# tigert1998/ray-tracing-cuda

Measured on AMD Instinct MI355X. Metric: Mrays/s, higher is better.
Workload: dtype f32

## Files before the change

### ray-tracing-cuda_amd/csrc/capi.hip

```cpp
#include <hip/hip_runtime.h>
#include <dlfcn.h>
#include <rccl/rccl.h>
#include <string.h>

#include <algorithm>
#include <cmath>
#include <cstdlib>
#include <mutex>
#include <string>
#include <unordered_map>

#include "../../include/rtmi.h"
#include "kernels.h"
#include "scene.h"
#include "xorwow.h"

using namespace rtmi;

static thread_local std::string g_err;
static int fail(int code, const std::string &msg) {
  g_err = msg;
  return code;
}
static int hip_fail(hipError_t e, const char *what) {
// ... 332 lines not shown
  if (!s || !pos || !look_at || !up) return fail(RTMI_ERR_INVALID, "null argument");
  camera_pinhole(*S(s), v3(pos), v3(look_at), v3(up), fov, aspect);
  S(s)->committed = false;
  return RTMI_OK;
}
int rtmi_camera_defocus(rtmi_scene *s, const float pos[3], const float look_at[3], const float up[3], double fov,
                        double aspect, double aperture, double focus_distance) {
  if (!s || !pos || !look_at || !up) return fail(RTMI_ERR_INVALID, "null argument");
  camera_defocus(*S(s), v3(pos), v3(look_at), v3(up), fov, aspect, aperture, focus_distance);
  S(s)->committed = false;
  return RTMI_OK;
}
int rtmi_camera_raw(rtmi_scene *s, const float pos[3], const float llc[3], const float horiz[3], const float vert[3]) {
  if (!s || !pos || !llc || !horiz || !vert) return fail(RTMI_ERR_INVALID, "null argument");
  camera_raw(*S(s), v3(pos), v3(llc), v3(horiz), v3(vert));
  S(s)->committed = false;
  return RTMI_OK;
}
int rtmi_camera_set(rtmi_scene *s, const float f[21], int is_defocus, double lens_radius) {
  if (!s || !f) return fail(RTMI_ERR_INVALID, "null argument");
  CameraDev &c = S(s)->cam;
  c.position = v3(f), c.llc = v3(f + 3), c.horizontal = v3(f + 6), c.vertical = v3(f + 9);
  c.u = v3(f + 12), c.v = v3(f + 15);
  S(s)->cam_w = v3(f + 18);
  c.defocus = is_defocus ? 1 : 0;
  c.lens_radius = (float)lens_radius;
  S(s)->has_camera = true;
  S(s)->committed = false;
  return RTMI_OK;
}
int rtmi_camera_update(rtmi_scene *s, const float f[21], int is_defocus, double lens_radius) {
  if (!s || !f) return fail(RTMI_ERR_INVALID, "null argument");
  if (!all_finite(f, 21)) return fail(RTMI_ERR_INVALID, "non-finite camera float");
  Scene *sc = S(s);
  const bool committed = sc->committed;
  if (int rc = rtmi_camera_set(s, f, is_defocus, lens_radius)) return rc;
  if (committed) {
    sc->dev.cam = sc->cam;
    sc->features = sc->cam.defocus ? sc->features | F_DEFOCUS : sc->features & ~(uint32_t)F_DEFOCUS;
    sc->committed = true;
  }
  return RTMI_OK;
}
int rtmi_camera_get(const rtmi_scene *s, float out[21]) {
  if (!s || !out || !S(s)->has_camera) return fail(RTMI_ERR_INVALID, "scene has no camera");
  const CameraDev &c = S(s)->cam;
  const V3 vs[7] = {c.position, c.llc, c.horizontal, c.vertical, c.u, c.v, S(s)->cam_w};
  for (int i = 0; i < 7; i++) out[i * 3] = vs[i].x, out[i * 3 + 1] = vs[i].y, out[i * 3 + 2] = vs[i].z;
  return RTMI_OK;
}

int rtmi_scene_commit(rtmi_scene *sp) {
  if (!sp) return fail(RTMI_ERR_INVALID, "null scene");
  Scene *s = S(sp);
  if (s->list_counts.size() != 1) return fail(RTMI_ERR_INVALID, "a nested list is still open (rtmi_list_end missing)");
  static_assert(RTMI_MAX_MATERIALS == kMaxMats, "rtmi.h and scene_dev.h disagree on the material limit");
  if (s->mats.size() > (size_t)RTMI_MAX_MATERIALS)
    return fail(RTMI_ERR_CAPACITY, "more than RTMI_MAX_MATERIALS (2^24) materials: a triangle's material field has 24 bits");
  if (rtmi_device_count() <= 0) return fail(RTMI_ERR_NO_DEVICE, "no HIP device: librtmi has no CPU fallback");
  free_device(s);
  std::string err = s->flatten();
  if (!err.empty()) return fail(RTMI_ERR_INVALID, err);
  HIP_TRY(hipGetDevice(&s->device));
  s->tex_recs.clear();
  for (const HostTex &t : s->texs) {
    if (!t.image) continue;
    void *d = nullptr;
    size_t pitch = 0;
    HIP_TRY(hipMallocPitch(&d, &pitch, (size_t)t.w * 4, (size_t)t.h));
    s->dev_allocs.push_back(d);
    HIP_TRY(hipMemcpy2D(d, pitch, t.rgba.data(), (size_t)t.w * 4, (size_t)t.w * 4, (size_t)t.h,
                        hipMemcpyHostToDevice));
    TexRec r{};
    r.rgba = reinterpret_cast<const uint8_t *>(d);
    r.height = t.h, r.width = t.w, r.pitch = (int64_t)pitch;
    s->tex_recs.push_back(r);
  }
  SceneDev d{};
  int rc;
  if ((rc = upload(s, s->runs, &d.runs))) return rc;
  if ((rc = upload(s, s->spheres, &d.spheres))) return rc;
  if ((rc = upload(s, s->tris, &d.tris))) return rc;
  if ((rc = upload(s, s->pair_boxes, &d.pair_boxes))) return rc;
  if ((rc = upload(s, s->pair_pts, &d.pair_pts))) return rc;
  if ((rc = upload(s, s->tri_nrm, &d.tri_nrm))) return rc;
  if ((rc = upload(s, s->sph_groups, &d.sph_groups))) return rc;
  if ((rc = upload(s, s->sph_members, &d.sph_members))) return rc;
  d.sph_mag = s->sph_mag;
  d.n_sph_groups = (int)s->sph_groups.size();
  if ((rc = upload(s, s->bvh_recs, &d.bvhs))) return rc;
  if ((rc = upload(s, s->nodes, &d.nodes))) return rc;
  if ((rc = upload(s, s->qnodes, &d.qnodes))) return rc;
  if ((rc = upload(s, s->leaf_paths, &d.leaf_paths))) return rc;
  if ((rc = upload(s, s->tops, &d.tops))) return rc;
  if ((rc = upload(s, s->faces, &d.faces))) return rc;
  if ((rc = upload(s, s->face_uv, &d.face_uv))) return rc;
#ifdef RTMI_CHECK_MARGINS
  if ((rc = upload(s, s->face_of_orig, &d.face_of_orig))) return rc;
#endif
  if ((rc = upload(s, s->mat_recs, &d.mats))) return rc;
  if ((rc = upload(s, s->tex_recs, &d.texs))) return rc;
  d.n_runs = (int)s->runs.size() - 4;
  d.n_pairs = (int)s->pair_pts.size();
  d.list_mag = s->list_mag;
  d.n_mats = (int)s->mat_recs.size();
  d.n_nodes = (int)s->nodes.size();
  d.n_leaf_paths = (int)s->leaf_paths.size();
  d.sub_reserve = s->sub_depth > 0 ? 3 * s->sub_depth + 3 + kMeshFaceSlack : 0;
  d.det_safe = 1;
  for (const HotTri &t : s->tris) {
    const double a = std::sqrt((double)t.e1[0] * t.e1[0] + (double)t.e1[1] * t.e1[1] + (double)t.e1[2] * t.e1[2]);
    const double b = std::sqrt((double)t.e2[0] * t.e2[0] + (double)t.e2[1] * t.e2[1] + (double)t.e2[2] * t.e2[2]);
    if (!(a * b <= 0x1p120)) d.det_safe = 0;
  }
  d.unsigned_colours = 1;
  for (const MatRec &m : s->mat_recs) {
    const float c[3] = {m.r, m.g, m.b};
    for (float x : c) {
      uint32_t bits;
      memcpy(&bits, &x, sizeof(bits));
      if (bits >> 31) d.unsigned_colours = 0;
    }
  }
  d.cam = s->cam;
  s->dev = d;
  QueryDev q{};
  if ((rc = upload(s, s->q_sphere_entry, &q.sphere_entry))) return rc;
  if ((rc = upload(s, s->q_pair_entry, &q.pair_entry))) return rc;
  if ((rc = upload(s, s->q_bvh_entry, &q.bvh_entry))) return rc;
  if ((rc = upload(s, s->q_face_input, &q.face_input))) return rc;
  q.sky_entry = s->q_sky_entry;
  s->qdev = q;
  void *c = nullptr;
  HIP_TRY(hipMalloc(&c, RTMI_COUNTER_WORDS * sizeof(unsigned long long) + 2 * render_params_bytes()));
  s->dev_allocs.push_back(c);
  HIP_TRY(hipMemset(c, 0, RTMI_COUNTER_WORDS * sizeof(unsigned long long)));
  s->d_counters = reinterpret_cast<unsigned long long *>(c);
  HIP_TRY(hipDeviceSynchronize());
  s->committed = true;
  return RTMI_OK;
}

static int flattened(const rtmi_scene *sp, Scene *tmp) {
  *tmp = *S(sp);
  tmp->dev_allocs.clear();
  const std::string err = tmp->flatten();
  return err.empty() ? RTMI_OK : fail(RTMI_ERR_INVALID, err);
}
int rtmi_scene_stats(const rtmi_scene *sp, int64_t out[8]) {
  if (!sp || !out) return fail(RTMI_ERR_INVALID, "null argument");
  Scene tmp;
  if (int rc = flattened(sp, &tmp)) return rc;
  out[0] = (int64_t)tmp.list_counts[0];
  out[1] = (int64_t)tmp.n_spheres;
  out[2] = (int64_t)tmp.n_pgrams;
  out[3] = (int64_t)tmp.n_triangles;
  out[4] = (int64_t)tmp.faces.size();
  out[5] = (int64_t)tmp.nodes.size();
  out[6] = (int64_t)tmp.mat_recs.size();
  out[7] = (int64_t)tmp.texs.size();
  return RTMI_OK;
}

int64_t rtmi_scene_sliver_faces(const rtmi_scene *sp) {
  if (!sp) return fail(RTMI_ERR_INVALID, "null scene");
  Scene tmp;
  if (int rc = flattened(sp, &tmp)) return rc;
  return tmp.sliver_faces;
}

int64_t rtmi_scene_bytes_per_ray(const rtmi_scene *sp) {
  if (!sp) return fail(RTMI_ERR_INVALID, "null scene");
  Scene tmp;
  if (int rc = flattened(sp, &tmp)) return rc;
  return tmp.bytes_per_ray;
}

int64_t rtmi_frame_work_items(const rtmi_frame *f) {
  FrameDev d;
  if (!make_frame(f, &d)) return fail(RTMI_ERR_INVALID, frame_why("bad frame"));
  return d.items;
}
int64_t rtmi_frame_pixel_of(const rtmi_frame *f, int64_t q) {
  FrameDev d;
  if (!make_frame(f, &d) || q < 0 || q >= d.items) return -1;
  return frame_pixel_of(d, d.rank, q);
}
int rtmi_frame_pixel_map(const rtmi_frame *f, int64_t *out) {
  FrameDev d;
  if (!make_frame(f, &d) || !out) return fail(RTMI_ERR_INVALID, frame_why("bad frame"));
  for (int64_t q = 0; q < d.items; q++) out[q] = frame_pixel_of(d, d.rank, q);
  return RTMI_OK;
}
size_t rtmi_states_bytes(const rtmi_frame *f) {
  FrameDev d;
  if (!make_frame(f, &d)) return 0;
  return (size_t)d.items * RTMI_STATE_WORDS * sizeof(uint32_t);
}
size_t rtmi_tiles_bytes(const rtmi_frame *f) {
  FrameDev d;
  if (!make_frame(f, &d)) return 0;
  return (size_t)d.items * 3 * sizeof(float);
}

int rtmi_rng_init(uint64_t seed, const rtmi_frame *f, void *d_states, void *stream) {
  FrameDev d;
  if (!make_frame(f, &d) || !d_states) return fail(RTMI_ERR_INVALID, frame_why("bad rng_init arguments"));
  if (rtmi_device_count() <= 0) return fail(RTMI_ERR_NO_DEVICE, "no HIP device: librtmi has no CPU fallback");
  uint32_t *jump = nullptr;
  int rc = device_jump(&jump);
  if (rc) return rc;
  HIP_TRY(launch_rng_init(seed, d, jump, reinterpret_cast<uint32_t *>(d_states), (hipStream_t)stream));
  return RTMI_OK;
}
int rtmi_rng_init_n(uint64_t seed, uint64_t first, int64_t n, void *d_states, void *stream) {
  if (n < 0 || n > (int64_t)INT32_MAX || (n > 0 && !d_states) || first > (1ull << kJumpBits) ||
      (uint64_t)n > (1ull << kJumpBits) - first)
    return fail(RTMI_ERR_INVALID, "bad rng_init_n arguments (n < 0, n above 2^31 - 1, first + n above 2^40, or null states)");
  if (n == 0) return RTMI_OK;
  if (rtmi_device_count() <= 0) return fail(RTMI_ERR_NO_DEVICE, "no HIP device: librtmi has no CPU fallback");
  uint32_t *jump = nullptr;
  int rc = device_jump(&jump);
  if (rc) return rc;
  FrameDev d{};
  d.items = n;
  HIP_TRY(launch_rng_init(seed, d, jump, reinterpret_cast<uint32_t *>(d_states), (hipStream_t)stream, (int64_t)first));
  return RTMI_OK;
}
int rtmi_rng_host_state(uint64_t seed, uint64_t subsequence, uint32_t state[RTMI_STATE_WORDS]) {
  if (!state) return fail(RTMI_ERR_INVALID, "null state");
  Rng r = host_rng_init(seed, subsequence);
  state[0] = r.d, state[1] = r.v0, state[2] = r.v1, state[3] = r.v2, state[4] = r.v3, state[5] = r.v4;
  return RTMI_OK;
}
float rtmi_rng_host_random_float(float mn, float mx, uint32_t state[RTMI_STATE_WORDS]) {
  Rng r{state[0], state[1], state[2], state[3], state[4], state[5]};
  float x = rng_range(mn, mx, r);
  state[0] = r.d, state[1] = r.v0, state[2] = r.v1, state[3] = r.v2, state[4] = r.v3, state[5] = r.v4;
  return x;
}
int rtmi_rng_set_state(const rtmi_frame *f, void *d_states, int64_t q, const uint32_t state[RTMI_STATE_WORDS],
                       void *stream) {
  FrameDev d;
  if (!make_frame(f, &d) || !d_states || !state || q < 0 || q >= d.items)
    return fail(RTMI_ERR_INVALID, "bad rng_set_state arguments");
  uint32_t *base = reinterpret_cast<uint32_t *>(d_states);
  for (int w = 0; w < RTMI_STATE_WORDS; w++)
    HIP_TRY(hipMemcpyAsync(base + (size_t)w * d.items + q, &state[w], sizeof(uint32_t), hipMemcpyHostToDevice,
                           (hipStream_t)stream));
  HIP_TRY(hipStreamSynchronize((hipStream_t)stream));
  return RTMI_OK;
}
int rtmi_rng_get_state(const rtmi_frame *f, const void *d_states, int64_t q, uint32_t state[RTMI_STATE_WORDS],
                       void *stream) {
  FrameDev d;
  if (!make_frame(f, &d) || !d_states || !state || q < 0 || q >= d.items)
    return fail(RTMI_ERR_INVALID, "bad rng_get_state arguments");
  const uint32_t *base = reinterpret_cast<const uint32_t *>(d_states);
// ... 795 lines not shown
```

### ray-tracing-cuda_amd/csrc/closest_hit.h

```cpp
#pragma once

#ifdef RTMI_CHECK_MARGINS
__device__ inline bool aabb_hit_reference(const BvhNode &nd, V3 o, V3 d, double t_from, double t_to) {
  const float oo[3] = {o.x, o.y, o.z}, dd[3] = {d.x, d.y, d.z};
  for (int i = 0; i < 3; i++) {
    if (dd[i] == 0.f) continue;
    for (int s = 0; s < 2; s++) {
      const float tf = ((s == 0 ? nd.mn[i] : nd.mx[i]) - oo[i]) / dd[i];
      const double t = (double)tf;
      if (t != t || fabs(t) == (double)INFINITY) continue;
      if (!(t_from <= t && t <= t_to)) continue;
      const float pt[3] = {oo[0] + (float)t * dd[0], oo[1] + (float)t * dd[1], oo[2] + (float)t * dd[2]};
      bool inside = true;
      for (int a = 0; a < 3; a++)
        if (a != i && !(nd.mn[a] <= pt[a] && pt[a] <= nd.mx[a])) inside = false;
      if (inside) return true;
    }
  }
  return false;
}
template <typename T>
__device__ inline bool bvh_reference_walk(const SceneDev &sc, const BvhRec &br, V3 o, V3 d, T &t_to, int &face, float &fu,
                                          float &fv) {
  int stk_node[kRefDepthMax + 2], stk_first[kRefDepthMax + 2], stk_n[kRefDepthMax + 2];
  int sp = 1;
  stk_node[0] = br.root, stk_first[0] = 0, stk_n[0] = br.n_faces;
  bool hit = false;
  while (sp > 0) {
    sp--;
    const int node = stk_node[sp], first = stk_first[sp], n = stk_n[sp];
    const BvhNode nd = sc.nodes[node];
    if (node != br.root && !aabb_hit_reference(nd, o, d, 1e-3, (double)t_to)) continue;
    if (nd.right < 0) {
      for (int i = 0; i < n; i++) {
        const int fi = sc.face_of_orig[br.face_base + first + i];
        const FaceRec &f = sc.faces[fi];
        float t = 0.f, u = 0.f, v = 0.f;
        if (tri_test<T>(mk(f.p0[0], f.p0[1], f.p0[2]), mk(f.e1[0], f.e1[1], f.e1[2]), mk(f.e2[0], f.e2[1], f.e2[2]), o, d,
                        t_to, t, u, v))
          t_to = (T)t, face = fi, fu = u, fv = v, hit = true;
      }
    } else if (sp + 2 <= kRefDepthMax + 2) {
      const int mid = (n - 1) / 2;
      stk_node[sp] = nd.right, stk_first[sp] = first + mid + 1, stk_n[sp] = n - mid - 1;
      stk_node[sp + 1] = nd.left, stk_first[sp + 1] = first, stk_n[sp + 1] = mid + 1;
      sp += 2;
    }
  }
  return hit;
}
#endif

template <uint32_t F, bool OCC = false, uint32_t M = 0>
__device__ __forceinline__ Hit closest_hit(const SceneDev &sc, const BvhNode *s_nodes, int lds_nodes, const int *s_paths,
                                           int lds_paths, const float4 *s_pairs, int *ll, uint16_t *cands, int *wl,
                                           unsigned long long *overflow, V3 o, V3 d, bool live, bool count_work
#ifdef RTMI_STATS
                                           , MeshStats &st
#endif
                                           , double t_start = INFINITY, double t_stop = INFINITY, bool *uncertain = nullptr
) {
  constexpr bool DT = (F & F_SPHERE) != 0;
  typedef typename TSel<DT>::type T;
  bool ok = false;
  T t_to = OCC ? (T)t_start : (T)INFINITY;
#define RTMI_DECIDED (OCC && ok && t_to <= (T)t_stop)
  uint32_t win = ID_NONE;
  int32_t aux = 0;
  int32_t work = 0;
  float bu = 0.f, bv = 0.f;

  double sa = 0.0, sa2 = 0.0;
  float saf = 0.f;
  if (F & F_SPHERE) {
    float la = len3(d);
    saf = la * la;
    sa = (double)saf;
    sa2 = 2 * sa;
  }

  const int lane = (int)(threadIdx.x & 63u);
  const bool det_safe = (M & PIN_DET_SAFE) || sc.det_safe != 0;
  const bool cull_list = (F & F_TRIS) && ((M & PIN_LDS_TABLES) || (ll != nullptr && sc.n_pairs >= kCullMinPairs));
  V3 cull_inv = splat(0.f), cull_klo = splat(0.f), cull_khi = splat(0.f);
  if ((F & F_TRIS) && cull_list) {
    const float ix = __builtin_amdgcn_rcpf(d.x), iy = __builtin_amdgcn_rcpf(d.y), iz = __builtin_amdgcn_rcpf(d.z);
    cull_inv = mk(fabsf(d.x) < 1e-30f ? copysignf(1e30f, d.x) : ix, fabsf(d.y) < 1e-30f ? copysignf(1e30f, d.y) : iy,
                  fabsf(d.z) < 1e-30f ? copysignf(1e30f, d.z) : iz);
    const float delta = MESH_DIST_SLACK * (fmaxf(fmaxf(fabsf(o.x), fabsf(o.y)), fabsf(o.z)) + sc.list_mag);
    cull_klo = mk(-(o.x + delta) * cull_inv.x, -(o.y + delta) * cull_inv.y, -(o.z + delta) * cull_inv.z);
    cull_khi = mk(-(o.x - delta) * cull_inv.x, -(o.y - delta) * cull_inv.y, -(o.z - delta) * cull_inv.z);
  }

  for (int ri = 0; ri < sc.n_runs; ri++) {
    if (OCC) {
      live = live && !RTMI_DECIDED;
      if (__builtin_amdgcn_ballot_w64(live) == 0ull) break;
    }
    const i32x4 rv = load_run(sc.runs, ri);
    Run run;
    run.kind = rv[0], run.first = rv[1], run.count = rv[2], run.pad = rv[3];
    if (live && run.kind == RUN_SKY) {
      const T ts = (T)1e9f;
      bool hit = ts <= t_to;
      bool acc = hit && (!ok || ts < t_to);
      ok = ok || acc;
      t_to = acc ? ts : t_to;
      win = acc ? make_id(RUN_SKY, 0) : win;
    }
    if ((F & F_TRIS) && run.kind == RUN_TRIS && cull_list) {
      const int pair0 = run.first >> 1;
      const float lo0 = T_FROM_F * kTimeLo;
      for (int c0 = 0; c0 < run.count; c0 += 32) {
        if (OCC && __builtin_amdgcn_ballot_w64(live && !RTMI_DECIDED) == 0ull) break;
        const int nc = run.count - c0 < 32 ? run.count - c0 : 32;
        const float hi0 = (float)t_to * kTimeHi + kTimeAbs;
        uint32_t mask = 0u;
        RTMI_STAT2(const unsigned long long tc0 = stat_now();)
#define RTMI_CULL_PAIR(bx)                                                                                                      \
  {                                                                                                                             \
    const float t0x = __builtin_fmaf(bx[0], cull_inv.x, cull_klo.x), t1x = __builtin_fmaf(bx[3], cull_inv.x, cull_khi.x); \
    const float t0y = __builtin_fmaf(bx[1], cull_inv.y, cull_klo.y), t1y = __builtin_fmaf(bx[4], cull_inv.y, cull_khi.y); \
    const float t0z = __builtin_fmaf(bx[2], cull_inv.z, cull_klo.z), t1z = __builtin_fmaf(bx[5], cull_inv.z, cull_khi.z); \
    const float en = fmaxf(fmaxf(fminf(t0x, t1x), fminf(t0y, t1y)), fminf(t0z, t1z));                                            \
    const float le = fminf(fminf(fmaxf(t0x, t1x), fmaxf(t0y, t1y)), fmaxf(t0z, t1z));                                            \
    cull_step(mask, fmaxf(lo0, en), fminf(hi0, le));                                                                            \
  }
        f32x8 A = load_pair_box(sc.pair_boxes, pair0 + c0), B;
        int i = 0;
        for (; i + 1 < nc; i += 2) {
          __builtin_amdgcn_s_waitcnt(0xc07f);
          __builtin_amdgcn_sched_barrier(0);
          B = load_pair_box(sc.pair_boxes, pair0 + c0 + i + 1);
          __builtin_amdgcn_sched_barrier(0);
          RTMI_CULL_PAIR(A)
          __builtin_amdgcn_s_waitcnt(0xc07f);
          __builtin_amdgcn_sched_barrier(0);
          A = load_pair_box(sc.pair_boxes, pair0 + c0 + i + 2);
          __builtin_amdgcn_sched_barrier(0);
          RTMI_CULL_PAIR(B)
        }
        if (i < nc) {
          __builtin_amdgcn_s_waitcnt(0xc07f);
          __builtin_amdgcn_sched_barrier(0);
          RTMI_CULL_PAIR(A)
        }
#undef RTMI_CULL_PAIR
        mask = __brev(mask) >> (32 - nc);
        if (!live) mask = 0u;
        if (OCC && RTMI_DECIDED) mask = 0u;
        RTMI_STAT2(const unsigned long long tc1 = stat_now(); st.cyc[5] += tc1 - tc0;)
        RTMI_STAT(st.cull_bits += (unsigned)__popcll(__builtin_amdgcn_ballot_w64(true)) * 0u; { unsigned pc = __builtin_popcount(mask); for (int off = 32; off > 0; off >>= 1) pc += __shfl_down(pc, off); st.cull_bits += __builtin_amdgcn_readfirstlane(pc); } st.cull_rays += (unsigned)__popcll(__builtin_amdgcn_ballot_w64(true));)
#ifndef RTMI_OWN_FIRST
#define RTMI_OWN_FIRST 1
#endif
#if RTMI_OWN_FIRST
        if (__builtin_amdgcn_ballot_w64(mask != 0u) != 0ull) {
          if (mask != 0u) {
            const int bit = __builtin_ctz(mask);
            mask &= mask - 1u;
            const size_t pidx = (size_t)(pair0 + c0 + bit) * 4;
            float4 qa, qb, qc, qd;
            if ((M & PIN_LDS_TABLES) || s_pairs != nullptr) {
              const float4 *pp = s_pairs + pidx;
              qa = load_lds<float4>(pp), qb = load_lds<float4>(pp + 1), qc = load_lds<float4>(pp + 2), qd = load_lds<float4>(pp + 3);
            } else {
              const float4 *pp = reinterpret_cast<const float4 *>(sc.pair_pts) + pidx;
              qa = load_global<float4>(pp), qb = load_global<float4>(pp + 1), qc = load_global<float4>(pp + 2), qd = load_global<float4>(pp + 3);
            }
            const V3 p0 = mk(qa.x, qa.y, qa.z), p1 = mk(qa.w, qb.x, qb.y), p2 = mk(qb.z, qb.w, qc.x), p3 = mk(qc.y, qc.z, qc.w);
            float ta = 0.f, ua = 0.f, va = 0.f, tb = 0.f, ub = 0.f, vb = 0.f;
            const V3 e1 = p1 - p0, e2 = p2 - p0;
            const bool hit_a = tri_test_flat<T>(p0, e1, e2, cross3(d, e2), o, d, t_to, ta, ua, va, det_safe);
            bool hit_b = false;
            if (__float_as_int(qd.x) & PAIR_SECOND) {
              const V3 e1b = p2 - p1, e2b = p3 - p1;
              hit_b = tri_test_flat<T>(p1, e1b, e2b, cross3(d, e2b), o, d, t_to, tb, ub, vb, det_safe) && !hit_a;
            }
            const float t = hit_a ? ta : tb;
            const bool acc = (hit_a || hit_b) && (!ok || (T)t < t_to);
            ok = ok || acc;
            t_to = acc ? (T)t : t_to;
            win = acc ? make_id(RUN_TRIS, run.first + 2 * (c0 + bit) + (hit_a ? 0 : 1)) : win;
            if (F & F_TEX) {
              bu = acc ? (hit_a ? ua : ub) : bu;
              bv = acc ? (hit_a ? va : vb) : bv;
            }
          }
        }
        if (OCC && RTMI_DECIDED) mask = 0u;
#endif
        {
          constexpr int RW = (F & F_TEX) ? 6 : 2;
          int *tasks = ll + 64 * 8, *results = ll + 64 * 8 + kListTasks(F);
          const int cnt = __builtin_popcount(mask);
          const int base = wave_prefix_excl(cnt);
          if (cnt != 0) {
            int *rr = ll + lane * 8;
            int w3 = 0, w7 = 0;
            if (DT) {
              const double td = (double)t_to;
              w3 = __double2loint(td), w7 = __double2hiint(td);
            } else {
              w3 = __float_as_int((float)t_to);
            }
            *reinterpret_cast<int4 *>(rr) = make_int4(__float_as_int(o.x), __float_as_int(o.y), __float_as_int(o.z), w3);
            *reinterpret_cast<int4 *>(rr + 4) = make_int4(__float_as_int(d.x), __float_as_int(d.y), __float_as_int(d.z), w7);
          }
          bool todo = cnt != 0;
          while (__builtin_amdgcn_ballot_w64(todo) != 0ull) {
            RTMI_STAT(st.cull_iters++;)
            const int lo_t = __builtin_amdgcn_readlane(base, __builtin_ctzll(__builtin_amdgcn_ballot_w64(todo)));
            const bool now = todo && base + cnt - lo_t <= kListTasks(F);
            const int n_now = __builtin_amdgcn_readlane(base + cnt, 63 - __builtin_clzll(__builtin_amdgcn_ballot_w64(now))) - lo_t;
            if (now) {
              int k = base - lo_t;
              for (uint32_t m = mask; m != 0u; m &= m - 1u) tasks[k++] = (lane << 5) | __builtin_ctz(m);
            }
            wave_lds_fence();
            for (int t0 = 0; t0 < n_now; t0 += 64) {
              const int ti = t0 + lane;
              if (ti < n_now) {
                const int w = tasks[ti];
                const int *orr = ll + (w >> 5) * 8;
                const float4 r0 = *reinterpret_cast<const float4 *>(orr), r1 = *reinterpret_cast<const float4 *>(orr + 4);
                T t0_to;
                if (DT) {
                  t0_to = (T)__hiloint2double(__float_as_int(r1.w), __float_as_int(r0.w));
                } else {
                  t0_to = (T)r0.w;
                }
                const V3 ro = mk(r0.x, r0.y, r0.z), rd = mk(r1.x, r1.y, r1.z);
                const size_t pidx = (size_t)(pair0 + c0 + (w & 31)) * 4;
                float4 qa, qb, qc, qd;
                if ((M & PIN_LDS_TABLES) || s_pairs != nullptr) {
                  const float4 *pp = s_pairs + pidx;
                  qa = load_lds<float4>(pp), qb = load_lds<float4>(pp + 1), qc = load_lds<float4>(pp + 2), qd = load_lds<float4>(pp + 3);
                } else {
                  const float4 *pp = reinterpret_cast<const float4 *>(sc.pair_pts) + pidx;
                  qa = load_global<float4>(pp), qb = load_global<float4>(pp + 1), qc = load_global<float4>(pp + 2), qd = load_global<float4>(pp + 3);
                }
                const V3 p0 = mk(qa.x, qa.y, qa.z), p1 = mk(qa.w, qb.x, qb.y), p2 = mk(qb.z, qb.w, qc.x), p3 = mk(qc.y, qc.z, qc.w);
                float ta = 0.f, ua = 0.f, va = 0.f, tb = 0.f, ub = 0.f, vb = 0.f;
                const V3 e1 = p1 - p0, e2 = p2 - p0;
                const bool hit_a = tri_test_flat<T>(p0, e1, e2, cross3(rd, e2), ro, rd, t0_to, ta, ua, va, det_safe);
                bool hit_b = false;
                if (__float_as_int(qd.x) & PAIR_SECOND) {
                  const V3 e1b = p2 - p1, e2b = p3 - p1;
                  hit_b = tri_test_flat<T>(p1, e1b, e2b, cross3(rd, e2b), ro, rd, t0_to, tb, ub, vb, det_safe);
                }
                int *res = results + ti * RW;
                res[0] = hit_a ? __float_as_int(ta) : (int)0xffffffff;
                res[1] = hit_b ? __float_as_int(tb) : (int)0xffffffff;
                if (F & F_TEX) {
                  res[2] = __float_as_int(ua), res[3] = __float_as_int(va), res[4] = __float_as_int(ub), res[5] = __float_as_int(vb);
                }
              }
            }
            wave_lds_fence();
            RTMI_STAT2(const unsigned long long tc2 = stat_now();)
            if (now) {
              int k = base - lo_t;
              for (uint32_t m = mask; m != 0u; m &= m - 1u, k++) {
                const int tri = run.first + 2 * (c0 + __builtin_ctz(m));
                const int *res = results + k * RW;
                const int ia = res[0], ib = res[1];
                const float ta = __int_as_float(ia), tb = __int_as_float(ib);
                const bool hit_a = ia != (int)0xffffffff && (T)ta <= t_to;
                const bool hit_b = !hit_a && ib != (int)0xffffffff && (T)tb <= t_to;
                const float t = hit_a ? ta : tb;
                const bool acc = (hit_a || hit_b) && (!ok || (T)t < t_to);
                ok = ok || acc;
                t_to = acc ? (T)t : t_to;
                win = acc ? make_id(RUN_TRIS, tri + (hit_a ? 0 : 1)) : win;
                if (F & F_TEX) {
                  bu = acc ? __int_as_float(hit_a ? res[2] : res[4]) : bu;
                  bv = acc ? __int_as_float(hit_a ? res[3] : res[5]) : bv;
                }
              }
              todo = false;
            }
            wave_lds_fence();
            RTMI_STAT2(st.cyc[7] += stat_now() - tc2;)
          }
        }
        RTMI_STAT2(st.cyc[6] += stat_now() - tc1;)
      }
    } else if ((F & F_TRIS) && live && run.kind == RUN_TRIS) {
      const HotTri *base = sc.tris + run.first;
      f32x16 A = load_hot_tri(base, 0);
      for (int i = 0; i < run.count; i++) {
        if (OCC && __builtin_amdgcn_ballot_w64(!RTMI_DECIDED) == 0ull) break;
        __builtin_amdgcn_s_waitcnt(0xc07f);
        __builtin_amdgcn_sched_barrier(0);
        const f32x16 B = load_hot_tri(base, 2 * i + 1);
        __builtin_amdgcn_sched_barrier(0);
        float t = 0.f, u = 0.f, v = 0.f;
        const V3 pv_a = cross3(d, mk(A[6], A[7], A[8]));
        const bool hit_a = tri_test_flat<T>(mk(A[0], A[1], A[2]), mk(A[3], A[4], A[5]), mk(A[6], A[7], A[8]), pv_a, o, d,
                                            t_to, t, u, v, det_safe);
        {
          bool acc = hit_a && (!ok || (T)t < t_to);
          ok = ok || acc;
          t_to = acc ? (T)t : t_to;
          win = acc ? make_id(RUN_TRIS, run.first + 2 * i) : win;
          if (F & F_TEX) {
            bu = acc ? u : bu;
            bv = acc ? v : bv;
          }
        }
        __builtin_amdgcn_s_waitcnt(0xc07f);
        __builtin_amdgcn_sched_barrier(0);
        A = load_hot_tri(base, 2 * i + 2);
        __builtin_amdgcn_sched_barrier(0);
        if (__float_as_int(B[13]) & TRI_SECOND) {
          V3 pv_b = pv_a;
          if (!(__float_as_int(B[13]) & TRI_SAME_E2)) pv_b = cross3(d, mk(B[6], B[7], B[8]));
          bool hit_b = tri_test_flat<T>(mk(B[0], B[1], B[2]), mk(B[3], B[4], B[5]), mk(B[6], B[7], B[8]), pv_b, o, d,
                                        t_to, t, u, v, det_safe);
          hit_b = hit_b && !hit_a;
          bool acc = hit_b && (!ok || (T)t < t_to);
          ok = ok || acc;
          t_to = acc ? (T)t : t_to;
          win = acc ? make_id(RUN_TRIS, run.first + 2 * i + 1) : win;
          if (F & F_TEX) {
            bu = acc ? u : bu;
            bv = acc ? v : bv;
          }
        }
      }
    }
    bool grouped_done = false;
    if ((F & F_SGROUP) && run.kind == RUN_SPHERE && run.pad >= 0 && cands != nullptr) {
      const int n_groups = (run.count + kSphGroupSize - 1) / kSphGroupSize;
      uint16_t *my_cands = cands + lane * kSphCand;
      int *tasks = ll + 64 * 8, *results = ll + 64 * 8 + kListTasks(F);
      int ccnt = 0;
      bool have = false;
      double best_v = 0.0;
// ... 435 lines not shown
```

### ray-tracing-cuda_amd/csrc/kernels.h

```cpp
#pragma once
#include <hip/hip_runtime.h>
#include <stdint.h>

#include "../../include/rtmi.h"
#include "scene_dev.h"

#define RTMI_KERNEL_MAX_DEPTH 64

namespace rtmi {

int64_t frame_pixel_of(const FrameDev &fr, int rank, int64_t q);

hipError_t launch_rng_init(uint64_t seed, const FrameDev &fr, const uint32_t *d_jump, uint32_t *d_states,
                           hipStream_t stream, int64_t first = -1);

uint32_t pick_variant(uint32_t features);
int render_occupancy(uint32_t variant, const SceneDev &sc, const FrameDev &fr, int threads, bool fast_path = false);
struct RenderTuning {
  int schedule;
  int blocks_per_cu;
  int threads;
  int sparse_stride;
  int exclusive;
  int outlier_x10;
  int head_pct[3];
  int probe_spp;
  int promote;
  int first_pass;
  int cost_probe;
  int lane_stride;
  int plan;
  int prio_every;
  int fast_path;
  int head_classes;
  int first_prio;
  int fetch_batch, fetch_batch_first;
};

enum : uint32_t {
  PIN_NIBBLE_IDS = 1u << 0,
  PIN_LDS_TABLES = 1u << 1,
  PIN_UNSIGNED = 1u << 2,
  PIN_DET_SAFE = 1u << 3,
  PIN_POW2_FRAME = 1u << 4,
  PIN_EVERY_LANE = 1u << 5,
  PIN_PRIORITIES = 1u << 6,
  PIN_CHAINS = 1u << 7,
  PIN_QUEUE = 1u << 8,
};
constexpr uint32_t kFastCommon = PIN_NIBBLE_IDS | PIN_LDS_TABLES | PIN_UNSIGNED | PIN_DET_SAFE | PIN_POW2_FRAME |
                                 PIN_EVERY_LANE | PIN_PRIORITIES;
constexpr uint32_t kFastChains = kFastCommon | PIN_CHAINS;
constexpr uint32_t kFastQueue = kFastCommon | PIN_QUEUE;
struct FastPathFacts {
  int enabled;
  uint32_t variant;
  int n_mats;
  int mats_in_lds;
  int pairs_in_lds;
  int unsigned_colours;
  int det_safe;
  int width, height;
  int lane_stride;
  int priorities;
  int chains;
  int resumed;
  int tile_cost;
};
uint32_t fast_path_mode(const FastPathFacts &f);
FastPathFacts fast_path_facts(uint32_t variant, const SceneDev &sc, const FrameDev &fr, int threads, int enabled);
struct SchedPlan {
  const uint32_t *tile_order = nullptr;
  uint32_t *visit_counts = nullptr;
  const uint32_t *sparse_items = nullptr;
  const uint32_t *head_list = nullptr;
  const uint32_t *probe_marks = nullptr;
  int probe_spp = 2;
  uint32_t *prio_tab = nullptr;
  const uint32_t *tile_cost = nullptr;
  const int32_t *chain_next = nullptr;
  const uint32_t *chain_fut = nullptr;
  const int32_t *chain_first = nullptr;
  uint32_t *claims = nullptr;
  int plan_simds = 0, plan_rounds = 0;
};
size_t render_params_bytes();
hipError_t launch_render(uint32_t variant, const SceneDev &sc, const FrameDev &fr, uint32_t *d_states, float *d_out,
                         uint32_t *d_ray_counts, unsigned long long *d_counters, const SchedPlan &plan, bool probe,
                         uint32_t fast, int blocks, int threads, const RenderTuning &tune, void *d_params, hipStream_t stream);
constexpr int kHeadCap = 16384;
hipError_t launch_tile_order(uint32_t *d_ray_counts, int n_tiles, uint32_t *d_cost, uint32_t *d_meta,
                             uint32_t *d_order, uint32_t *d_head, uint32_t sparse_cap, int grid_waves, int outlier_x10,
                             const int head_pct[3], hipStream_t stream);

hipError_t launch_quarter_order(const uint32_t *d_order, const uint32_t *d_work, const uint32_t *d_rays, int n_tiles,
                                uint32_t *d_qcost, uint32_t *d_qsorted, uint32_t *d_qmax, uint32_t *d_qmap, hipStream_t stream);

hipError_t launch_chain_plan(const uint32_t *d_order, const uint32_t *d_cost, int n_tiles, int simds, int rounds, int spp,
                             int probe_spp, int32_t *d_first, int32_t *d_next, uint32_t *d_fut, hipStream_t stream);

hipError_t launch_untile(const FrameDev &fr, const float *d_tiles, float *d_image, hipStream_t stream);
hipError_t launch_untile_u32(const FrameDev &fr, const uint32_t *d_tiles, uint32_t *d_image, hipStream_t stream);
hipError_t launch_post(float *d_img, int64_t n, int spp, hipStream_t stream);
uint32_t pick_query_variant(uint32_t features);
hipError_t launch_query(uint32_t variant, const SceneDev &sc, const QueryDev &qd, int n_cu, int64_t n, const float *d_o,
                        const float *d_d, const float *d_t_max, int32_t *d_hits, unsigned long long *d_abandoned,
                        unsigned long long *d_check, hipStream_t stream);
hipError_t launch_occlusion(uint32_t variant, const SceneDev &sc, const float near_lo[3], const float near_hi[3],
                            float near_short, int n_cu, int64_t n, const float *d_o, const float *d_d,
                            const float *d_t_max, uint8_t *d_occluded, unsigned long long *d_counts,
                            unsigned long long *d_check, hipStream_t stream);
constexpr size_t kCallParamsOffset = 256;
hipError_t launch_trace(uint32_t variant, const SceneDev &sc, bool tex_layers, int n_cu, int64_t n, int max_depth,
                        const float *d_o, const float *d_d, uint32_t *d_states, float *d_radiance,
                        uint32_t *d_ray_counts, unsigned long long *d_work, hipStream_t stream);
hipError_t launch_budget(uint32_t variant, const SceneDev &sc, bool tex_layers, int n_cu, const FrameDev &fr,
                         const uint32_t *d_budget, uint32_t *d_states, float *d_sum, float *d_sq, uint32_t *d_samples,
                         uint32_t *d_ray_counts, const FeatureBufs *feat, unsigned long long *d_work, hipStream_t stream);
hipError_t launch_resolve_features(const FrameDev &fr, const FeatureBufs &sums, const uint32_t *d_samples,
                                   const FeatureBufs &out, hipStream_t stream);
hipError_t launch_budget_plan(const FrameDev &fr, int min_samples, int max_samples, int step, float tolerance, float floor,
                              const float *d_sum, const float *d_sq, const uint32_t *d_samples, uint32_t *d_budget,
                              unsigned long long *d_totals, hipStream_t stream);
hipError_t launch_resolve(const FrameDev &fr, const float *d_sum, const uint32_t *d_samples, int post, float *d_tiles,
                          hipStream_t stream);
hipError_t launch_resolve_variance(const FrameDev &fr, const float *d_sum, const float *d_sq, const uint32_t *d_samples,
                                   float *d_var, hipStream_t stream);
struct DenoiseCall {
  int height, width, iterations, normal_squarings, demodulate;
  float sigma_color, sigma_depth;
  const float *color, *variance, *albedo, *normal, *depth, *alpha;
  float *out, *out_variance;
  void *scratch;
};
size_t denoise_scratch_bytes(int height, int width);
hipError_t launch_denoise(const DenoiseCall &d, hipStream_t stream);
struct AccumulateCall {
  int height, width;
  float normal_min, depth_tolerance, min_blend;
  float e[3], h[3], v[3], p[3];
  float prev_p[3], r[3][3];
  const float *color, *variance, *normal, *depth, *alpha;
  const void *history_in;
  void *history_out;
  float *out, *out_variance, *out_length;
};
size_t history_bytes(int height, int width);
hipError_t launch_accumulate(const AccumulateCall &c, hipStream_t stream);
#ifdef RTMI_STATS
hipError_t copy_wave_stats(unsigned long long *host, size_t bytes);
#endif
#ifdef RTMI_CHECK_MARGINS
hipError_t launch_add_one(unsigned long long *d_word, hipStream_t stream);
// ... 5 lines not shown
```

### ray-tracing-cuda_amd/csrc/kernels.hip

```cpp
#include <hip/hip_runtime.h>
#include <stdint.h>

#include "kernels.h"

#include <cstdlib>
#include <iterator>
#include <type_traits>
#include "scene_dev.h"
#include "vec.h"
#include "xorwow.h"

namespace rtmi {

__host__ __device__ __forceinline__ int64_t frame_pixel_of_rank(const FrameDev &fr, int rank, int64_t q) {
  int64_t lt = q >> 6;
  int w = (int)(q & 63);
  int64_t gt = lt * fr.world + rank;
  if (gt >= fr.n_tiles) return -1;
  int ty = (int)(gt / fr.tiles_x), tx = (int)(gt % fr.tiles_x);
  int i = ty * 8 + (w >> 3), j = tx * 8 + (w & 7);
  if (i >= fr.height || j >= fr.width) return -1;
  return (int64_t)i * fr.width + j;
}

// ... 388 lines not shown
      rx = 0x80000000u + (rx >> (8 + (sh & 15))), ry = 0x80000000u - (ry >> (8 + ((sh >> 4) & 15))),
      rz = 0x80000000u + (rz >> (8 + ((sh >> 8) & 15)));
    const float cx = rng_pm1_of(rx), cy = rng_pm1_of(ry), cz = rng_pm1_of(rz);
    const float sum = cx * cx + cy * cy + cz * cz;
    if (sum > BALL_S_MAX) continue;
    const float l = sqrtf(sum);
    if (!(l >= DIV3_RN_LO)) continue;
    const float y = rcp_rn(l);
    const float v[3] = {cx, cy, cz};
    for (int k = 0; k < 3; k++) {
      const float ref = v[k] / l;
      const float q0 = v[k] * y;
      if (__float_as_uint(ref) != __float_as_uint(div_rn_core(v[k], l, y))) dv++;
      if (__float_as_uint(ref) != __float_as_uint(__builtin_fmaf(__builtin_fmaf(-l, q0, v[k]), y, q0))) dv1++;
    }
  }
  if (in_domain) atomicAdd(&bad[0], in_domain);
  if (outside) atomicAdd(&bad[1], outside);
  if (pm1) atomicAdd(&bad[2], pm1);
  if (u01) atomicAdd(&bad[3], u01);
  if (sq) atomicAdd(&bad[4], sq);
  if (dv) atomicAdd(&bad[5], dv);
  if (dv1) atomicAdd(&bad[6], dv1);
}
#ifdef RTMI_STATS
hipError_t copy_wave_stats(unsigned long long *host, size_t bytes) {
  return hipMemcpyFromSymbol(host, HIP_SYMBOL(g_wave_stats), bytes);
}
#endif
hipError_t launch_arithmetic_selftest(unsigned long long *d_bad, hipStream_t stream) {
  hipLaunchKernelGGL(arithmetic_selftest, dim3(4096), dim3(256), 0, stream, d_bad, -1.f, 1.f, 0.f, 1.f);
  return hipGetLastError();
}
#ifdef RTMI_CHECK_MARGINS
__global__ void add_one_kernel(unsigned long long *word) { atomicAdd(word, 1ull); }
hipError_t launch_add_one(unsigned long long *d_word, hipStream_t stream) {
  hipLaunchKernelGGL(add_one_kernel, dim3(1), dim3(1), 0, stream, d_word);
  return hipGetLastError();
}
#endif

static inline int64_t cdiv(int64_t a, int64_t b) { return (a + b - 1) / b; }

hipError_t launch_rng_init(uint64_t seed, const FrameDev &fr, const uint32_t *d_jump, uint32_t *d_states,
                           hipStream_t stream, int64_t first) {
  if (fr.items == 0) return hipSuccess;
  hipLaunchKernelGGL(rng_init_kernel, dim3((unsigned)cdiv(fr.items, 256)), dim3(256), 0, stream, seed, fr, first, d_jump,
                     d_states);
  return hipGetLastError();
}

static bool plain_list_scan() {
  static const bool v = [] {
    const char *e = getenv("RTMI_PLAIN_LIST");
    return e && atoi(e) != 0;
  }();
  return v;
}

static LaunchCfg make_cfg(uint32_t variant, const SceneDev &sc, const FrameDev &fr, int threads, size_t *lds_bytes,
                          bool mats_in_lds = true, bool id_stack = true, bool tex_layers = true) {
  LaunchCfg lc{};
  lc.threads = threads;
  lc.tile_order = nullptr;
  lc.lds_mats = mats_in_lds && sc.n_mats <= kLdsMats ? sc.n_mats : 0;
  lc.wide_ids = sc.n_mats > 256 ? 1 : sc.n_mats <= 16 ? 2 : 0;
  size_t off = ((size_t)lc.lds_mats * sizeof(MatRec) + 15) & ~(size_t)15;
  lc.stack_off = (int32_t)off;
  const size_t levels = (size_t)(fr.max_depth > 0 ? fr.max_depth : 1);
  size_t stack = (variant & F_TEX) && tex_layers ? levels * threads * 4 : (lc.wide_ids == 2 ? (levels + 1) / 2 : levels) * threads * (lc.wide_ids == 1 ? 2 : 1);
  if (!id_stack) stack = 0;
  size_t noff = (off + stack + 15) & ~(size_t)15;
  lc.nodes_off = (int32_t)noff;
  lc.lds_nodes = (variant & F_BVH) ? (sc.n_nodes < kLdsNodes ? sc.n_nodes : kLdsNodes) : 0;
  size_t paoff = (noff + (size_t)lc.lds_nodes * sizeof(BvhNode) + 15) & ~(size_t)15;
  lc.paths_off = (int32_t)paoff;
  lc.lds_paths = (variant & F_BVH) ? (sc.n_leaf_paths < kLdsPaths ? sc.n_leaf_paths : kLdsPaths) : 0;
  size_t soff = (paoff + (size_t)lc.lds_paths * sizeof(int32_t) + 15) & ~(size_t)15;
  lc.mesh_off = (int32_t)soff;
  size_t poff = soff + ((variant & F_BVH) ? (size_t)(threads / 64) * kMeshWaveWords * sizeof(int) : 0);
  const bool cull = (variant & F_TRIS) && sc.n_pairs >= kCullMinPairs && !plain_list_scan();
  const bool staged = cull && sc.n_pairs <= kLdsPairs;
  lc.pairs_off = staged ? (int32_t)poff : -1;
  size_t noff2 = (poff + (staged ? (size_t)sc.n_pairs * sizeof(PairPts) : 0) + 15) & ~(size_t)15;
  lc.nrm_off = staged ? (int32_t)noff2 : -1;
  size_t loff = (noff2 + (staged ? (size_t)sc.n_pairs * 2 * sizeof(TriNrm) : 0) + 15) & ~(size_t)15;
  const bool groups = (variant & F_SGROUP) && sc.n_sph_groups > 0;
  const bool share = cull || groups;
  lc.list_off = share ? (int32_t)loff : -1;
  size_t coff = loff + (share ? (size_t)(threads / 64) * kListWaveWords(variant) * sizeof(int) : 0);
  lc.cand_off = groups ? (int32_t)coff : -1;
  *lds_bytes = coff + (groups ? (size_t)threads * (kSphCand * sizeof(uint16_t) + sizeof(int)) : 0);
  if (groups && mats_in_lds && lc.lds_mats > 0 && *lds_bytes * (size_t)(1024 / threads) > 160 * 1024) {
    size_t without = 0;
    const LaunchCfg alt = make_cfg(variant, sc, fr, threads, &without, false, id_stack, tex_layers);
    if (without * (size_t)(1024 / threads) <= 160 * 1024) {
      *lds_bytes = without;
      return alt;
    }
  }
  return lc;
}

template <auto Kernel>
static hipError_t dynamic_lds(size_t lds) {
  const void *k = reinterpret_cast<const void *>(Kernel);
  if (lds > 64 * 1024) {
    const hipError_t e = hipFuncSetAttribute(k, hipFuncAttributeMaxDynamicSharedMemorySize, (int)lds);
    if (e != hipSuccess) return e;
  }
  static const hipError_t no_static = [k] {
    hipFuncAttributes a{};
    const hipError_t e = hipFuncGetAttributes(&a, k);
    return e != hipSuccess ? e : a.sharedSizeBytes == 0 ? hipSuccess : hipErrorInvalidConfiguration;
  }();
  return no_static;
}

constexpr uint32_t kVariants[] = {0u, F_TRIS, F_SPHERE, F_TRIS | F_SPHERE, F_SPHERE | F_SGROUP, F_TRIS | F_SPHERE | F_SGROUP,
                                  F_TRIS | F_BVH, F_TRIS | F_SPHERE | F_TEX, F_ALL};
constexpr uint32_t kQueryVariants[] = {F_TEX, F_TRIS | F_TEX, F_SPHERE | F_TEX, F_TRIS | F_SPHERE | F_TEX,
                                       F_SPHERE | F_SGROUP | F_TEX, F_TRIS | F_SPHERE | F_SGROUP | F_TEX,
                                       F_TRIS | F_BVH | F_TEX, F_ALL & ~F_DEFOCUS};
template <size_t N>
static uint32_t pick_listed(const uint32_t (&list)[N], uint32_t features) {
  for (const uint32_t v : list)
    if ((features & ~v) == 0) return v;
  return list[N - 1];
}
uint32_t pick_variant(uint32_t features) { return pick_listed(kVariants, features); }
uint32_t pick_query_variant(uint32_t features) {
  return pick_listed(kQueryVariants, (features & ~(uint32_t)F_DEFOCUS) | F_TEX);
}
template <const auto &List, size_t I = 0, class R, class Fn>
static R with_listed(uint32_t variant, R otherwise, Fn &&f) {
  if constexpr (I == std::size(List)) return otherwise;
  else if (variant == List[I]) return f(std::integral_constant<uint32_t, List[I]>());
  else return with_listed<List, I + 1>(variant, otherwise, f);
}

uint32_t fast_path_mode(const FastPathFacts &f) {
  const auto pow2 = [](int v) { return v > 0 && (v & (v - 1)) == 0 && v <= (1 << 20); };
  const bool common = f.enabled != 0 && f.variant == (uint32_t)F_TRIS && f.n_mats >= 1 && f.n_mats <= 16 && f.mats_in_lds != 0 &&
                      f.pairs_in_lds != 0 && f.unsigned_colours != 0 && f.det_safe != 0 && pow2(f.width) && pow2(f.height) &&
                      f.lane_stride == 1 && f.priorities != 0;
  if (!common) return 0u;
  if (!f.chains) return kFastQueue;
  return f.resumed && f.tile_cost ? kFastChains : 0u;
}
FastPathFacts fast_path_facts(uint32_t variant, const SceneDev &sc, const FrameDev &fr, int threads, int enabled) {
  size_t lds = 0;
  const LaunchCfg lc = make_cfg(variant, sc, fr, threads, &lds);
  FastPathFacts f{};
  f.enabled = enabled, f.variant = variant, f.n_mats = sc.n_mats, f.mats_in_lds = lc.lds_mats > 0 && lc.wide_ids == 2;
  f.pairs_in_lds = lc.pairs_off >= 0 && lc.nrm_off >= 0 && lc.list_off >= 0;
  f.unsigned_colours = sc.unsigned_colours, f.det_safe = sc.det_safe, f.width = fr.width, f.height = fr.height;
  return f;
}

template <auto Kernel>
static hipError_t kernel_occupancy(int threads, size_t lds, int *per_cu) {
  *per_cu = 0;
  if (lds > 160 * 1024) return hipErrorInvalidConfiguration;
  hipError_t e = dynamic_lds<Kernel>(lds);
  if (e == hipSuccess) e = hipOccupancyMaxActiveBlocksPerMultiprocessor(per_cu, Kernel, threads, lds);
  if (e != hipSuccess) *per_cu = 0;
  return e;
}
struct LaunchAt {
  int blocks, threads;
  size_t lds;
  hipStream_t stream;
};
template <auto Kernel, class P>
static hipError_t launch_block(const LaunchAt &at, const P &block, P *d_block) {
  const hipError_t e = dynamic_lds<Kernel>(at.lds);
  if (e != hipSuccess) return e;
  hipLaunchKernelGGL(params_write_kernel<P>, dim3(1), dim3(64), 0, at.stream, block, d_block);
  hipLaunchKernelGGL(Kernel, dim3(at.blocks), dim3(at.threads), at.lds, at.stream, (const P *)d_block);
  return hipGetLastError();
}
int render_occupancy(uint32_t variant, const SceneDev &sc, const FrameDev &fr, int threads, bool fast_path) {
  return with_listed<kVariants>(variant, 0, [&](auto v) {
    constexpr uint32_t F = decltype(v)::value;
    size_t lds = 0;
    (void)make_cfg(F, sc, fr, threads, &lds);
    if (threads > RTMI_MAX_THREADS(F)) return 0;
    int nb = 0;
    (void)kernel_occupancy<render_kernel<F>>(threads, lds, &nb);
    if constexpr (F == (uint32_t)F_TRIS) {
      if (fast_path) {
        int nc = 0, nq = 0;
        (void)kernel_occupancy<render_kernel<F, kFastChains>>(threads, lds, &nc);
        (void)kernel_occupancy<render_kernel<F, kFastQueue>>(threads, lds, &nq);
        nb = nb < nc ? nb : nc, nb = nb < nq ? nb : nq;
      }
    }
    return nb;
  });
}

static int image_order_batch(int samples, int cap) {
  const int per_atomic = samples < 32 ? 256 / (samples > 0 ? samples : 1) : 64 / samples;
  return per_atomic < 1 ? 1 : per_atomic > cap ? cap : per_atomic;
}

hipError_t launch_render(uint32_t variant, const SceneDev &sc, const FrameDev &fr, uint32_t *d_states, float *d_out,
                         uint32_t *d_ray_counts, unsigned long long *d_counters, const SchedPlan &plan, bool probe,
                         uint32_t fast, int blocks, int threads, const RenderTuning &tune, void *d_params, hipStream_t stream) {
  return with_listed<kVariants>(variant, hipErrorInvalidValue, [&](auto v) {
    constexpr uint32_t F = decltype(v)::value;
    size_t lds = 0;
    LaunchCfg lc = make_cfg(F, sc, fr, threads, &lds);
    lc.tile_order = plan.tile_order;
    lc.visit_counts = plan.visit_counts;
    lc.sparse_items = plan.sparse_items;
    lc.head_list = plan.head_list;
    lc.probe_marks = plan.probe_marks;
    lc.sparse_stride = tune.sparse_stride;
    lc.exclusive = tune.exclusive;
    lc.probe_spp = plan.probe_spp;
    lc.promote = tune.promote;
    lc.lane_stride = tune.lane_stride > 0 ? tune.lane_stride : 1;
    lc.prio_tab = plan.prio_tab;
    lc.tile_cost = plan.tile_cost;
    lc.rate_scale = 1.f / (64.f * (float)(plan.probe_spp > 0 ? plan.probe_spp : 1));
    lc.chain_next = (F & F_BVH) || lc.prio_tab == nullptr ? nullptr : plan.chain_next;
    lc.chain_fut = plan.chain_fut, lc.chain_first = plan.chain_first, lc.claims = plan.claims;
    lc.plan_simds = plan.plan_simds, lc.plan_rounds = plan.plan_rounds;
    lc.prio_every = tune.prio_every > 0 ? tune.prio_every : 16;
    {
      const int samples = fr.k_end - fr.k_begin > 0 ? fr.k_end - fr.k_begin : 1;
      const int by_length = 4096 / samples < 1 ? 1 : 4096 / samples;
      lc.fetch_batch = probe && samples <= 4 ? tune.fetch_batch_first : plan.tile_order != nullptr ? std::min(by_length, tune.fetch_batch) : image_order_batch(samples, 16);
    }
    RenderParams rp;
    rp.sc = sc, rp.fr = fr, rp.lc = lc;
    rp.states = d_states, rp.out = d_out, rp.ray_counts = d_ray_counts, rp.counters = d_counters;
    RenderParams *dp = reinterpret_cast<RenderParams *>(d_params);
    const LaunchAt at{blocks, threads, lds, stream};
// ... 299 lines not shown
```

### ray-tracing-cuda_amd/csrc/mesh_search.h

```cpp
#pragma once

__device__ __forceinline__ int lane_rank(unsigned long long mask) {
  return (int)__builtin_amdgcn_mbcnt_hi((unsigned)(mask >> 32), __builtin_amdgcn_mbcnt_lo((unsigned)mask, 0u));
}
__device__ __forceinline__ int wave_prefix_excl(int v) {
  int s = v;
  s += __builtin_amdgcn_update_dpp(0, s, 0x111, 0xf, 0xf, true);
  s += __builtin_amdgcn_update_dpp(0, s, 0x112, 0xf, 0xf, true);
  s += __builtin_amdgcn_update_dpp(0, s, 0x114, 0xf, 0xf, true);
  s += __builtin_amdgcn_update_dpp(0, s, 0x118, 0xf, 0xf, true);
  s += __builtin_amdgcn_update_dpp(0, s, 0x142, 0xa, 0xf, false);
  s += __builtin_amdgcn_update_dpp(0, s, 0x143, 0xc, 0xf, false);
  return s - v;
}
__device__ __forceinline__ void wave_lds_fence() {
  __builtin_amdgcn_fence(__ATOMIC_ACQ_REL, "wavefront");
  __builtin_amdgcn_wave_barrier();
}
__device__ __forceinline__ float ubyte_f32(uint32_t x, int byte) { return (float)((x >> (8 * byte)) & 0xffu); }

#ifndef MESH_DIST_SLACK
#define MESH_DIST_SLACK kDistSlack
#endif

struct NodeFrame {
  float ka[3], kb[3], idq[3];
};
__device__ __forceinline__ void node_frame(uint4 w0, float4 r0, float4 r2, float mag, NodeFrame &f) {
  const float delta = MESH_DIST_SLACK * (fmaxf(fmaxf(fabsf(r0.x), fabsf(r0.y)), fabsf(r0.z)) + mag);
  const float oo[3] = {r0.x, r0.y, r0.z}, ii[3] = {r2.x, r2.y, r2.z};
  const float org[3] = {__uint_as_float(w0.x), __uint_as_float(w0.y), __uint_as_float(w0.z)};
#ifdef RTMI_NO_SLACK_EXP
  const int sk = 0;
#else
  const int sk = (int)w0.w >> 24;
#endif
#pragma unroll
  for (int a = 0; a < 3; a++) {
    const int ex = (int)(int8_t)((w0.w >> (8 * a)) & 0xffu);
    const float oq = ldexpf(oo[a] - org[a], -ex);
    const float rho = ldexpf(delta, sk - ex);
    f.idq[a] = __builtin_amdgcn_fmed3f(ldexpf(ii[a], ex), -1e35f, 1e35f);
    f.ka[a] = -(oq + rho) * f.idq[a];
    f.kb[a] = -(oq - rho) * f.idq[a];
  }
}
__device__ __forceinline__ bool child_box_hit(const NodeFrame &f, float qlx, float qly, float qlz, float qhx, float qhy,
                                              float qhz, float lo0, float hi0) {
  const float ql[3] = {qlx, qly, qlz}, qh[3] = {qhx, qhy, qhz};
  float en = -INFINITY, le = INFINITY;
#pragma unroll
  for (int a = 0; a < 3; a++) {
    const float tl = __builtin_fmaf(ql[a], f.idq[a], f.ka[a]);
    const float th = __builtin_fmaf(qh[a], f.idq[a], f.kb[a]);
    en = fmaxf(en, fminf(tl, th));
    le = fminf(le, fmaxf(tl, th));
  }
  const float lo = fmaxf(lo0, __builtin_fmaf(-fabsf(en), kSlabTimeRel, en));
  const float hi = fminf(hi0, __builtin_fmaf(fabsf(le), kSlabTimeRel, le));
  return lo <= hi;
}

__device__ __forceinline__ void hit_list_insert(const SceneDev &sc, int *rr, uint32_t code, int face, int orig,
                                                float t) {
  const int cnt = rr[12];
  const uint32_t cut = (uint32_t)rr[13], lo_code = (uint32_t)rr[14];
  if (!(code >= lo_code && code < cut)) return;
  int found = -1, jmax = 0;
  uint32_t cmax = 0u;
#pragma unroll
  for (int j = 0; j < kHitSlots; j++) {
    if (j < cnt) {
      const uint32_t cj = (uint32_t)rr[16 + j * kHitWords];
      if (cj == code) found = j;
      if (cj >= cmax) cmax = cj, jmax = j;
    }
  }
  int slot = -1;
  if (found >= 0) {
    const float tj = __int_as_float(rr[16 + found * kHitWords + 2]);
    bool better = t < tj;
    if (t == tj) better = orig > sc.faces[rr[16 + found * kHitWords + 1]].orig;
    if (better) slot = found;
  } else if (cnt < kHitSlots) {
    slot = cnt;
    rr[12] = cnt + 1;
  } else if (code > cmax) {
    rr[13] = (int)code;
  } else {
    rr[13] = (int)cmax;
    slot = jmax;
  }
  if (slot >= 0) {
    rr[16 + slot * kHitWords] = (int)code;
    rr[16 + slot * kHitWords + 1] = face;
    rr[16 + slot * kHitWords + 2] = __float_as_int(t);
  }
}

#ifdef RTMI_STATS
struct MeshStats {
  unsigned searches, node_steps, face_steps, nodes_popped, blocks_popped, insert_rounds, steps_hist[6];
  unsigned long long cull_bits, cull_rays, cull_iters;
  unsigned long long calib;
  unsigned long long cyc[11];
};
__device__ unsigned long long g_wave_stats[16384][16];
__device__ __forceinline__ unsigned long long stat_real() {
  __builtin_amdgcn_sched_barrier(0);
  unsigned long long t;
  asm volatile("s_waitcnt vmcnt(0) lgkmcnt(0)\n\ts_memtime %0\n\ts_waitcnt lgkmcnt(0)" : "=s"(t)::"memory");
  __builtin_amdgcn_sched_barrier(0);
  return t;
}
#if RTMI_STATS == 9
__device__ __forceinline__ unsigned long long stat_now() { return 0ull; }
#else
__device__ __forceinline__ unsigned long long stat_now() { return stat_real(); }
#endif
#define RTMI_STAT(x) x
#if RTMI_STATS == 2
#define RTMI_STAT2(x) x
#else
#define RTMI_STAT2(x)
#endif
#if RTMI_STATS == 3
#define RTMI_STAT3(x) x
#else
#define RTMI_STAT3(x)
#endif
#else
#define RTMI_STAT(x)
#define RTMI_STAT2(x)
#define RTMI_STAT3(x)
#endif

template <typename T, bool DT>
__device__ __forceinline__ void mesh_search(const SceneDev &sc, int sub_root, const BvhNode *top, float mag, int *wl,
                                            bool need, V3 o, V3 d, V3 inv_d, T bt_to, uint32_t lo_code,
                                            unsigned long long *overflow, bool count_work
#ifdef RTMI_STATS
                                            , MeshStats &st
#endif
) {
  const int lane = (int)(threadIdx.x & 63u);
  RTMI_STAT(st.searches++; unsigned my_steps = 0; const unsigned long long tset0 = stat_now();)
  int *stack = wl + 64 * kMeshRayWords;
  const float lo0 = T_FROM_F * kTimeLo;
  if (need) {
    int *rr = wl + lane * kMeshRayWords;
    int w3 = 0, w7 = 0;
    if (DT) {
      const double td = (double)bt_to;
      w3 = __double2loint(td), w7 = __double2hiint(td);
    } else {
      w3 = __float_as_int((float)bt_to);
    }
    *reinterpret_cast<int4 *>(rr + 0) = make_int4(__float_as_int(o.x), __float_as_int(o.y), __float_as_int(o.z), w3);
    *reinterpret_cast<int4 *>(rr + 4) = make_int4(__float_as_int(d.x), __float_as_int(d.y), __float_as_int(d.z), w7);
    *reinterpret_cast<int4 *>(rr + 8) = make_int4(__float_as_int(inv_d.x), __float_as_int(inv_d.y), __float_as_int(inv_d.z),
                                                  __float_as_int((float)bt_to * kTimeHi + kTimeAbs));
    *reinterpret_cast<int4 *>(rr + 12) = make_int4(0, (int)kCodeNone, (int)lo_code, 0);
  }
  const unsigned long long nm = __ballot(need);
  const int reserve = sc.sub_reserve;
  int sn = 0, sf = 0;
  if (__popcll(nm) <= kTopRays) {
    const BvhNode te = top[lane];
    const float far = (float)bt_to * kTimeHi + kTimeAbs;
    for (unsigned long long m = nm; m != 0ull; m &= m - 1ull) {
      const int rl = __builtin_ctzll(m);
      if (kMeshStackWords - sn - sf - reserve < kTopEntries) {
        if (lane == 0) stack[sn] = (rl << 26) | sub_root;
        sn++;
        continue;
      }
      const V3 ro = mk(__int_as_float(__builtin_amdgcn_readlane(__float_as_int(o.x), rl)),
                       __int_as_float(__builtin_amdgcn_readlane(__float_as_int(o.y), rl)),
                       __int_as_float(__builtin_amdgcn_readlane(__float_as_int(o.z), rl)));
      const V3 ri = mk(__int_as_float(__builtin_amdgcn_readlane(__float_as_int(inv_d.x), rl)),
                       __int_as_float(__builtin_amdgcn_readlane(__float_as_int(inv_d.y), rl)),
                       __int_as_float(__builtin_amdgcn_readlane(__float_as_int(inv_d.z), rl)));
      const float rfar = __int_as_float(__builtin_amdgcn_readlane(__float_as_int(far), rl));
      const float delta = ldexpf(MESH_DIST_SLACK * (fmaxf(fmaxf(fabsf(ro.x), fabsf(ro.y)), fabsf(ro.z)) + mag), te.right);
      const bool hit = te.left != -1 && slab_touch(te, delta, ro, ri, lo0, rfar);
      const bool pn = hit && te.left >= 0, pf = hit && te.left < 0;
// ... 266 lines not shown
```

### ray-tracing-cuda_amd/csrc/occlusion_body.h

```cpp
#pragma once

struct OcclusionParams {
  SceneDev sc;
  LaunchCfg lc;
  int64_t n;
  const float *origins, *dirs;
  const float *t_max;
  uint8_t *occluded;
  unsigned long long *counts;
  unsigned long long *check;
  int32_t dummy_off;
  float near_lo[3], near_hi[3];
  float near_short;
};

struct QueryLds {
  const BvhNode *s_nodes;
  const int *s_paths;
  const float4 *s_pairs;
  int *wl, *ll;
  uint16_t *cands;
};
template <uint32_t F>
__device__ __forceinline__ QueryLds query_stage(const SceneDev &sc, const LaunchCfg &lc, unsigned char *smem) {
  QueryLds q;
  q.s_nodes = reinterpret_cast<const BvhNode *>(smem + lc.nodes_off);
  q.wl = nullptr;
  if (F & F_BVH)
    q.wl = reinterpret_cast<int *>(smem + lc.mesh_off) + __builtin_amdgcn_readfirstlane((int)(threadIdx.x >> 6)) * kMeshWaveWords;
  q.s_pairs = nullptr;
  if ((F & F_TRIS) && lc.pairs_off >= 0) {
    q.s_pairs = reinterpret_cast<const float4 *>(smem + lc.pairs_off);
    const uint32_t *src = reinterpret_cast<const uint32_t *>(sc.pair_pts);
    uint32_t *dst = reinterpret_cast<uint32_t *>(smem + lc.pairs_off);
    for (int w = threadIdx.x; w < sc.n_pairs * 16; w += blockDim.x) dst[w] = src[w];
  }
  q.ll = nullptr;
  if ((F & (F_TRIS | F_SGROUP)) && lc.list_off >= 0)
    q.ll = reinterpret_cast<int *>(smem + lc.list_off) + __builtin_amdgcn_readfirstlane((int)(threadIdx.x >> 6)) * kListWaveWords(F);
  q.cands = nullptr;
  if ((F & F_SGROUP) && lc.cand_off >= 0)
    q.cands = reinterpret_cast<uint16_t *>(smem + lc.cand_off) +
              __builtin_amdgcn_readfirstlane((int)(threadIdx.x >> 6)) * (64 * kSphCand + 128);
  if ((F & F_BVH) && lc.lds_nodes > 0) {
    const uint32_t *src = reinterpret_cast<const uint32_t *>(sc.nodes);
    uint32_t *dst = reinterpret_cast<uint32_t *>(smem + lc.nodes_off);
    for (int w = threadIdx.x; w < lc.lds_nodes * 8; w += blockDim.x) dst[w] = src[w];
  }
  q.s_paths = reinterpret_cast<const int *>(smem + lc.paths_off);
  if ((F & F_BVH) && lc.lds_paths > 0) {
    int *dst = reinterpret_cast<int *>(smem + lc.paths_off);
    for (int w = threadIdx.x; w < lc.lds_paths; w += blockDim.x) dst[w] = sc.leaf_paths[w];
  }
  return q;
}

template <typename T>
__device__ __forceinline__ double occlusion_seed(float tm) {
  if (sizeof(T) == sizeof(float) || !(__builtin_fabsf(tm) < INFINITY)) return (double)tm;
  const int32_t b = __float_as_int(tm);
  const float up = tm == 0.f ? __int_as_float(1) : __int_as_float(tm > 0.f ? b + 1 : b - 1);
  double m = up == INFINITY ? (double)tm + 0x1p103 : ((double)tm + (double)up) * 0.5;
  if (!((float)m <= tm)) {
    const long long mb = __double_as_longlong(m);
    m = __longlong_as_double(m > 0.0 ? mb - 1 : mb + 1);
  }
  return m;
}

template <uint32_t F>
__device__ __forceinline__ void occlusion_body(const OcclusionParams &p) {
  constexpr bool DT = (F & F_SPHERE) != 0;
  typedef typename TSel<DT>::type T;
  extern __shared__ __attribute__((aligned(16))) unsigned char smem[];
  const SceneDev &sc = p.sc;
  const LaunchCfg &lc = p.lc;
  const QueryLds q = query_stage<F>(sc, lc, smem);
  unsigned long long *counts = p.counts;
  if (counts == nullptr) {
    counts = reinterpret_cast<unsigned long long *>(smem + p.dummy_off);
    if (threadIdx.x == 0) counts[0] = 0ull, counts[1] = 0ull;
  }
  __syncthreads();
#ifdef RTMI_STATS
  MeshStats st{};
#endif

  const int lane = (int)(threadIdx.x & 63u);
  const int64_t wave = (int64_t)blockIdx.x * (blockDim.x >> 6) + (threadIdx.x >> 6);
  const int64_t stride = (int64_t)gridDim.x * (blockDim.x >> 6) * 64;
  const bool all_lanes_in = (F & F_BVH) || ((F & F_TRIS) && q.ll != nullptr && sc.n_pairs >= kCullMinPairs) ||
                            ((F & F_SGROUP) && q.cands != nullptr);
  for (int64_t base = wave * 64; base < p.n; base += stride) {
    const int64_t i = base + lane;
    V3 o = splat(0.f), d = mk(0.f, 0.f, 1.f);
    bool live = false;
    float tm = INFINITY;
    if (i < p.n) {
      const V3 ro = mk(p.origins[i * 3], p.origins[i * 3 + 1], p.origins[i * 3 + 2]);
      const V3 rd = mk(p.dirs[i * 3], p.dirs[i * 3 + 1], p.dirs[i * 3 + 2]);
      live = finite3(ro) && finite3(rd) && (rd.x != 0.f || rd.y != 0.f || rd.z != 0.f);
      if (live) o = ro, d = rd;
      if (p.t_max != nullptr) tm = p.t_max[i];
    }
    d = unit3_rn(d);
    if (live && !(finite3(d) && (d.x != 0.f || d.y != 0.f || d.z != 0.f))) {
      live = false;
      o = splat(0.f), d = mk(0.f, 0.f, 1.f);
    }
    live = live && tm == tm;
    const double seed = occlusion_seed<T>(tm);
    const bool near = o.x >= p.near_lo[0] && o.x <= p.near_hi[0] && o.y >= p.near_lo[1] && o.y <= p.near_hi[1] &&
                      o.z >= p.near_lo[2] && o.z <= p.near_hi[2];
    const double start0 = near && !(tm < p.near_short) ? (double)INFINITY : seed;
    bool occ = false, unc = false;
#pragma nounroll
    for (int pass = 0; pass < 2; pass++) {
      const bool go = pass == 0 ? live : live && unc && !occ;
      if (pass == 1) {
        const unsigned long long nf = __builtin_amdgcn_ballot_w64(go);
        if (nf == 0ull) break;
        if (lane == 0) atomicAdd(&counts[1], (unsigned long long)__popcll(nf));
      }
      const double start = pass == 0 ? start0 : (double)INFINITY;
      Hit h = {};
      if (all_lanes_in)
        h = closest_hit<F, true>(sc, q.s_nodes, lc.lds_nodes, q.s_paths, lc.lds_paths, q.s_pairs, q.ll, q.cands, q.wl,
                                 counts, o, d, go, false
#ifdef RTMI_STATS
                                 , st
#endif
                                 , start, seed, &unc);
      else if (go)
        h = closest_hit<F, true>(sc, q.s_nodes, 0, q.s_paths, 0, q.s_pairs, nullptr, nullptr, nullptr, nullptr, o, d, true,
                                 false
#ifdef RTMI_STATS
                                 , st
#endif
                                 , start, seed, &unc);
      occ = occ || (go && h.ok && h.t <= tm);
    }
#ifdef RTMI_CHECK_MARGINS
    {
      Hit h2 = {};
      if (all_lanes_in)
        h2 = closest_hit<F>(sc, q.s_nodes, 0, q.s_paths, 0, nullptr, nullptr, nullptr, nullptr, nullptr, o, d, live, false
#ifdef RTMI_STATS
                            , st
#endif
        );
      else if (live)
        h2 = closest_hit<F>(sc, q.s_nodes, 0, q.s_paths, 0, nullptr, nullptr, nullptr, nullptr, nullptr, o, d, true, false
#ifdef RTMI_STATS
                            , st
#endif
        );
      const bool occ2 = live && h2.ok && h2.t <= tm;
      const unsigned long long na = __builtin_amdgcn_ballot_w64(i < p.n), nd = __builtin_amdgcn_ballot_w64(occ2 != occ);
      if (lane == 0 && p.check != nullptr) {
        if (na) atomicAdd(&p.check[0], (unsigned long long)__popcll(na));
        if (nd) atomicAdd(&p.check[1], (unsigned long long)__popcll(nd));
      }
    }
#endif
    if (i < p.n) p.occluded[i] = occ ? 1 : 0;
  }
}
```

### ray-tracing-cuda_amd/csrc/query_body.h

```cpp
#pragma once

struct QueryParams {
  SceneDev sc;
  QueryDev qd;
  LaunchCfg lc;
  int64_t n;
  const float *origins, *dirs;
  const float *t_max;
  int32_t *hits;
  unsigned long long *abandoned;
  unsigned long long *check;
  int32_t dummy_off;
};
constexpr size_t kQueryLdsExtra = 16;

struct QueryHit {
  float t, u, v;
  V3 n;
  int32_t mat, kind, entry, element;
};
template <uint32_t F>
__device__ __forceinline__ QueryHit resolve_hit(const SceneDev &sc, const QueryDev &qd, const Hit &h, V3 o, V3 d) {
  QueryHit r;
  r.t = INFINITY, r.u = 0.f, r.v = 0.f, r.n = splat(0.f);
  r.mat = -1, r.kind = QHIT_NONE, r.entry = -1, r.element = 0;
  if (!h.ok) return r;
  const uint32_t kind = h.win >> 29;
  const uint32_t index = h.win & ID_INDEX_MASK;
  r.t = h.t;
  if (kind == RUN_SKY) {
    r.kind = QHIT_SKY, r.entry = qd.sky_entry;
    return r;
  }
  if ((F & F_TRIS) && kind == RUN_TRIS) {
    const HotTri &tr = sc.tris[index];
    const V3 n = mk(tr.n[0], tr.n[1], tr.n[2]);
    r.n = dot3(d, n) < 0.f ? n : -n;
    r.mat = tr.mat;
    if (tr.flags & TRI_PGRAM) {
      const float w = (float)((1.0 - (double)h.u) - (double)h.v);
      if (!(tr.flags & TRI_SECOND)) {
        r.u = (0.f * w + 1.f * h.u) + 0.f * h.v;
        r.v = (1.f * w + 1.f * h.u) + 0.f * h.v;
      } else {
        r.u = (1.f * w + 0.f * h.u) + 1.f * h.v;
        r.v = (1.f * w + 0.f * h.u) + 0.f * h.v;
      }
    } else {
      r.u = h.u, r.v = h.v;
    }
    const int32_t info = qd.pair_entry[(index >> 1) * 2 + 1];
    r.entry = qd.pair_entry[(index >> 1) * 2];
    r.kind = info & 0xff;
    r.element = r.kind == QHIT_PARALLELEPIPED ? (info >> 8) : r.kind == QHIT_PARALLELOGRAM ? (int32_t)(index & 1u) : 0;
  }
  if ((F & F_SPHERE) && kind == RUN_SPHERE) {
    const SphereRec &sr = sc.spheres[index];
    const V3 p = o + h.t * d;
    r.n = unit3_rn(p - mk(sr.cx, sr.cy, sr.cz));
    r.mat = sr.mat;
    const float pi_f = 3.14159265358979323846264338327950288f;
    const float theta = acosf(-r.n.y);
    const float phi = atan2f(-r.n.z, r.n.x) + pi_f;
    r.u = phi / (2 * pi_f);
    r.v = theta / pi_f;
    r.kind = QHIT_SPHERE, r.entry = qd.sphere_entry[index];
  }
  if ((F & F_BVH) && kind == RUN_BVH) {
    const FaceRec &fc = sc.faces[index];
    const V3 n = unit3_rn(cross3(mk(fc.e1[0], fc.e1[1], fc.e1[2]), mk(fc.e2[0], fc.e2[1], fc.e2[2])));
    r.n = dot3(d, n) < 0.f ? n : -n;
    const BvhRec br = sc.bvhs[h.aux];
    r.mat = br.mat;
    if (br.has_uv) {
      const float *tc = sc.face_uv + (size_t)(br.face_base + fc.orig) * 6;
      const float w = (float)((1.0 - (double)h.u) - (double)h.v);
      r.u = (tc[0] * w + tc[2] * h.u) + tc[4] * h.v;
      r.v = (tc[1] * w + tc[3] * h.u) + tc[5] * h.v;
    }
    r.kind = QHIT_MESH, r.entry = qd.bvh_entry[h.aux], r.element = qd.face_input[index];
  }
  return r;
}

template <uint32_t F>
__device__ __forceinline__ void query_body(const QueryParams &qp) {
  extern __shared__ __attribute__((aligned(16))) unsigned char smem[];
  const SceneDev &sc = qp.sc;
  const LaunchCfg &lc = qp.lc;
  const BvhNode *s_nodes = reinterpret_cast<const BvhNode *>(smem + lc.nodes_off);
  int *wl = nullptr;
  if (F & F_BVH)
    wl = reinterpret_cast<int *>(smem + lc.mesh_off) + __builtin_amdgcn_readfirstlane((int)(threadIdx.x >> 6)) * kMeshWaveWords;
  const float4 *s_pairs = nullptr;
  if ((F & F_TRIS) && lc.pairs_off >= 0) {
    s_pairs = reinterpret_cast<const float4 *>(smem + lc.pairs_off);
    const uint32_t *src = reinterpret_cast<const uint32_t *>(sc.pair_pts);
    uint32_t *dst = reinterpret_cast<uint32_t *>(smem + lc.pairs_off);
    for (int w = threadIdx.x; w < sc.n_pairs * 16; w += blockDim.x) dst[w] = src[w];
  }
  int *ll = nullptr;
  if ((F & (F_TRIS | F_SGROUP)) && lc.list_off >= 0)
    ll = reinterpret_cast<int *>(smem + lc.list_off) + __builtin_amdgcn_readfirstlane((int)(threadIdx.x >> 6)) * kListWaveWords(F);
  uint16_t *cands = nullptr;
  if ((F & F_SGROUP) && lc.cand_off >= 0)
    cands = reinterpret_cast<uint16_t *>(smem + lc.cand_off) +
            __builtin_amdgcn_readfirstlane((int)(threadIdx.x >> 6)) * (64 * kSphCand + 128);
  if ((F & F_BVH) && lc.lds_nodes > 0) {
    const uint32_t *src = reinterpret_cast<const uint32_t *>(sc.nodes);
    uint32_t *dst = reinterpret_cast<uint32_t *>(smem + lc.nodes_off);
    for (int w = threadIdx.x; w < lc.lds_nodes * 8; w += blockDim.x) dst[w] = src[w];
  }
  const int *s_paths = reinterpret_cast<const int *>(smem + lc.paths_off);
  if ((F & F_BVH) && lc.lds_paths > 0) {
    int *dst = reinterpret_cast<int *>(smem + lc.paths_off);
    for (int w = threadIdx.x; w < lc.lds_paths; w += blockDim.x) dst[w] = sc.leaf_paths[w];
  }
  unsigned long long *abandoned = qp.abandoned;
  if (abandoned == nullptr) abandoned = reinterpret_cast<unsigned long long *>(smem + qp.dummy_off);
  __syncthreads();
#ifdef RTMI_STATS
  MeshStats st{};
#endif

  const int lane = (int)(threadIdx.x & 63u);
  const int64_t wave = (int64_t)blockIdx.x * (blockDim.x >> 6) + (threadIdx.x >> 6);
  const int64_t stride = (int64_t)gridDim.x * (blockDim.x >> 6) * 64;
  const bool all_lanes_in = (F & F_BVH) || ((F & F_TRIS) && ll != nullptr && sc.n_pairs >= kCullMinPairs) ||
                            ((F & F_SGROUP) && cands != nullptr);
  for (int64_t base = wave * 64; base < qp.n; base += stride) {
    const int64_t i = base + lane;
    V3 o = splat(0.f), d = mk(0.f, 0.f, 1.f);
    bool live = false;
    if (i < qp.n) {
      const V3 ro = mk(qp.origins[i * 3], qp.origins[i * 3 + 1], qp.origins[i * 3 + 2]);
      const V3 rd = mk(qp.dirs[i * 3], qp.dirs[i * 3 + 1], qp.dirs[i * 3 + 2]);
      live = finite3(ro) && finite3(rd) && (rd.x != 0.f || rd.y != 0.f || rd.z != 0.f);
      if (live) o = ro, d = rd;
    }
    d = unit3_rn(d);
    if (live && !(finite3(d) && (d.x != 0.f || d.y != 0.f || d.z != 0.f))) {
      live = false;
      o = splat(0.f), d = mk(0.f, 0.f, 1.f);
    }
    Hit h = {};
    if (all_lanes_in)
      h = closest_hit<F>(sc, s_nodes, lc.lds_nodes, s_paths, lc.lds_paths, s_pairs, ll, cands, wl, abandoned, o, d, live, false
#ifdef RTMI_STATS
                         , st
#endif
      );
    else if (live)
      h = closest_hit<F>(sc, s_nodes, 0, s_paths, 0, s_pairs, nullptr, nullptr, nullptr, nullptr, o, d, true, false
#ifdef RTMI_STATS
                         , st
#endif
      );
#ifdef RTMI_CHECK_MARGINS
    {
      Hit h2 = {};
      if (all_lanes_in)
        h2 = closest_hit<F>(sc, s_nodes, 0, s_paths, 0, nullptr, nullptr, nullptr, nullptr, nullptr, o, d, live, false
#ifdef RTMI_STATS
                            , st
#endif
        );
      else if (live)
        h2 = closest_hit<F>(sc, s_nodes, 0, s_paths, 0, nullptr, nullptr, nullptr, nullptr, nullptr, o, d, true, false
#ifdef RTMI_STATS
                            , st
#endif
        );
      const bool differs = live && (h2.ok != h.ok || (h.ok && (__float_as_uint(h2.t) != __float_as_uint(h.t) || h2.win != h.win ||
                                                             ((F & F_BVH) && h2.aux != h.aux))));
      const unsigned long long na = __builtin_amdgcn_ballot_w64(live), nd = __builtin_amdgcn_ballot_w64(differs);
      if (lane == 0 && qp.check != nullptr) {
        if (na) atomicAdd(&qp.check[0], (unsigned long long)__popcll(na));
        if (nd) atomicAdd(&qp.check[1], (unsigned long long)__popcll(nd));
      }
    }
#endif
    if (i < qp.n) {
      if (!live) h.ok = false;
      QueryHit r = resolve_hit<F>(sc, qp.qd, h, o, d);
      if (r.kind != QHIT_NONE && qp.t_max != nullptr && !(r.t <= qp.t_max[i])) {
        r.t = INFINITY, r.u = 0.f, r.v = 0.f, r.n = splat(0.f);
        r.mat = -1, r.kind = QHIT_NONE, r.entry = -1, r.element = 0;
      }
      int4 *out = reinterpret_cast<int4 *>(qp.hits + i * 12);
      out[0] = make_int4(__float_as_int(r.t), __float_as_int(r.u), __float_as_int(r.v), __float_as_int(r.n.x));
      out[1] = make_int4(__float_as_int(r.n.y), __float_as_int(r.n.z), r.mat, r.kind);
      out[2] = make_int4(r.entry, r.element, 0, 0);
    }
  }
}
```

### ray-tracing-cuda_amd/csrc/render_body.h

```cpp
#pragma once

struct LaunchCfg {
  int32_t lds_mats;
  int32_t wide_ids;
  int32_t stack_off;
  int32_t nodes_off;
  int32_t lds_nodes;
  int32_t mesh_off;
  int32_t exclusive;
  int32_t pairs_off;
  int32_t list_off;
  int32_t paths_off;
  int32_t lds_paths;
  int32_t threads;
  int32_t nrm_off;
  int32_t probe_spp;
  int32_t promote;
  int32_t cand_off;
  const uint32_t *tile_order;
  uint32_t *visit_counts;
  const uint32_t *head_list;
  const uint32_t *probe_marks;
  const uint32_t *sparse_items;
  int32_t sparse_stride;
// ... 47 lines not shown
      __hip_atomic_store(rowp + 14, simd + 1u, __ATOMIC_RELAXED, __HIP_MEMORY_SCOPE_AGENT);
    } else {
      while ((simd = __hip_atomic_load(rowp + 14, __ATOMIC_RELAXED, __HIP_MEMORY_SCOPE_AGENT)) == 0u) __builtin_amdgcn_s_sleep(2);
      simd -= 1u;
    }
  }
  round = (uint32_t)__builtin_amdgcn_readfirstlane((int)round), simd = (uint32_t)__builtin_amdgcn_readfirstlane((int)simd);
  return (round < (uint32_t)plan_rounds && simd < (uint32_t)plan_simds) ? (int)(round * (uint32_t)plan_simds + simd) : -1;
}
__device__ __forceinline__ void wave_priority_leave(uint32_t *tab) {
  const uint32_t hw = __builtin_amdgcn_s_getreg(0xF804), xcc = __builtin_amdgcn_s_getreg(0xF814);
  const uint32_t row = ((xcc & 15u) << 10) | (((hw >> 8) & 0xffu) << 2) | ((hw >> 4) & 3u);
  if ((threadIdx.x & 63u) == 0u && (hw & 15u) < 12u)
    __hip_atomic_store(tab + row * 16u + (hw & 15u), 0u, __ATOMIC_RELAXED, __HIP_MEMORY_SCOPE_AGENT);
}

__device__ __forceinline__ bool finite3(V3 v) {
  return __builtin_isfinite(v.x) && __builtin_isfinite(v.y) && __builtin_isfinite(v.z);
}

struct RenderParams {
  SceneDev sc;
  FrameDev fr;
  LaunchCfg lc;
  uint32_t *states;
  float *out;
  uint32_t *ray_counts;
  unsigned long long *counters;
};
struct RayBufs {
  const float *origins, *dirs;
};
struct BudgetBufs {
  const uint32_t *budget;
  float *sq;
  uint32_t *samples;
};
struct CallExtras {
  union {
    RayBufs rays;
    BudgetBufs px;
  };
  int32_t tex_layers;
  FeatureBufs feat;
};
struct CallParams {
  RenderParams rp;
  CallExtras ex;
};
template <class P>
__device__ __forceinline__ const P &in_constant(const P *p) {
  return *(const P *)(const RT_CONSTANT P *)(uintptr_t)p;
}

template <uint32_t F, bool RAYS = false, bool BUDGET = false, bool FEATURES = false, uint32_t M = 0>
__device__ __forceinline__ void render_body(const SceneDev &sc, const FrameDev &fr, const LaunchCfg &lc,
                                            uint32_t *__restrict__ states, float *__restrict__ out,
                                            uint32_t *__restrict__ ray_counts,
                                            unsigned long long *__restrict__ counters,
                                            const float *__restrict__ ray_o = nullptr,
                                            const float *__restrict__ ray_d = nullptr, bool tex_layers = true,
                                            const uint32_t *__restrict__ budget = nullptr,
                                            float *__restrict__ sq = nullptr, uint32_t *__restrict__ samples = nullptr,
                                            const FeatureBufs *feat = nullptr) {
  static_assert(!(RAYS && BUDGET), "one work-item source at a time");
  static_assert(!FEATURES || BUDGET, "the feature buffers belong to the budget mode");
  static_assert(M == 0 || (F == F_TRIS && !RAYS && !BUDGET), "the pins are the list-triangle render's");
  static_assert(!((M & PIN_CHAINS) && (M & PIN_QUEUE)), "a wave gets its work one way");
  constexpr bool FOLD4 = (M & (PIN_NIBBLE_IDS | PIN_LDS_TABLES | PIN_UNSIGNED)) == (PIN_NIBBLE_IDS | PIN_LDS_TABLES | PIN_UNSIGNED);
  constexpr bool QUEUE = RAYS || BUDGET;
  extern __shared__ __attribute__((aligned(16))) unsigned char smem[];
  MatRec *s_mats = reinterpret_cast<MatRec *>(smem);
  const uint32_t n_threads = (uint32_t)lc.threads;
  const uint32_t ids_shift = !(M & PIN_NIBBLE_IDS) && lc.wide_ids == 1 ? 1u : 0u;
  const bool nibble_ids = (M & PIN_NIBBLE_IDS) || lc.wide_ids == 2;
  auto ids_offset = [&](int level) -> uint32_t {
    return (uint32_t)lc.stack_off + (((uint32_t)level * n_threads + threadIdx.x) << ids_shift);
  };
  const BvhNode *s_nodes = reinterpret_cast<const BvhNode *>(smem + lc.nodes_off);
  int *wl = nullptr;
  if (F & F_BVH)
    wl = reinterpret_cast<int *>(smem + lc.mesh_off) +
         __builtin_amdgcn_readfirstlane((int)(threadIdx.x >> 6)) * kMeshWaveWords;
  const float4 *s_pairs = nullptr;
  if ((F & F_TRIS) && ((M & PIN_LDS_TABLES) || lc.pairs_off >= 0)) {
    s_pairs = reinterpret_cast<const float4 *>(smem + lc.pairs_off);
    const uint32_t *src = reinterpret_cast<const uint32_t *>(sc.pair_pts);
    uint32_t *dst = reinterpret_cast<uint32_t *>(smem + lc.pairs_off);
    for (int w = threadIdx.x; w < sc.n_pairs * 16; w += blockDim.x) dst[w] = src[w];
    const uint32_t *nsrc = reinterpret_cast<const uint32_t *>(sc.tri_nrm);
    uint32_t *ndst = reinterpret_cast<uint32_t *>(smem + lc.nrm_off);
    for (int w = threadIdx.x; w < sc.n_pairs * 8; w += blockDim.x) ndst[w] = nsrc[w];
  }
  const float4 *s_nrm = reinterpret_cast<const float4 *>(smem + ((M & PIN_LDS_TABLES) || lc.nrm_off >= 0 ? lc.nrm_off : 0));
  int *ll = nullptr;
  if ((F & (F_TRIS | F_SGROUP)) && ((M & PIN_LDS_TABLES) || lc.list_off >= 0))
    ll = reinterpret_cast<int *>(smem + lc.list_off) +
         __builtin_amdgcn_readfirstlane((int)(threadIdx.x >> 6)) * kListWaveWords(F);
  uint16_t *cands = nullptr;
  if ((F & F_SGROUP) && lc.cand_off >= 0)
    cands = reinterpret_cast<uint16_t *>(smem + lc.cand_off) +
            __builtin_amdgcn_readfirstlane((int)(threadIdx.x >> 6)) * (64 * kSphCand + 128);
  const bool mats_in_lds = (M & PIN_LDS_TABLES) || lc.lds_mats > 0;
  auto lds_rgb = [&](int m) -> V3 {
    const float4 c = load_lds<float4>(s_mats + m);
    return mk(c.x, c.y, c.z);
  };
  auto lds_byte = [&](uint32_t byte_offset) -> uint32_t {
    return *(const RT_LDS uint8_t *)(uintptr_t)byte_offset;
  };
  const bool fast_fold = FOLD4 || (mats_in_lds && lc.wide_ids != 1 && sc.unsigned_colours);
  if (mats_in_lds) {
    const uint32_t *src = reinterpret_cast<const uint32_t *>(sc.mats);
    uint32_t *dst = reinterpret_cast<uint32_t *>(s_mats);
    for (int w = threadIdx.x; w < lc.lds_mats * 8; w += blockDim.x) dst[w] = src[w];
  }
  if ((F & F_BVH) && lc.lds_nodes > 0) {
    const uint32_t *src = reinterpret_cast<const uint32_t *>(sc.nodes);
    uint32_t *dst = reinterpret_cast<uint32_t *>(smem + lc.nodes_off);
    for (int w = threadIdx.x; w < lc.lds_nodes * 8; w += blockDim.x) dst[w] = src[w];
  }
  const int *s_paths = reinterpret_cast<const int *>(smem + lc.paths_off);
  if ((F & F_BVH) && lc.lds_paths > 0) {
    int *dst = reinterpret_cast<int *>(smem + lc.paths_off);
    for (int w = threadIdx.x; w < lc.lds_paths; w += blockDim.x) dst[w] = sc.leaf_paths[w];
  }
  __syncthreads();

  const int64_t n_items = fr.items;
  const bool w_pow2 = (fr.width & (fr.width - 1)) == 0, h_pow2 = (fr.height & (fr.height - 1)) == 0;
  const double inv_w = 1.0 / (double)fr.width, inv_h = 1.0 / (double)fr.height;
  const bool f32_jitter = (M & PIN_POW2_FRAME) || (w_pow2 && h_pow2 && fr.width <= (1 << 20) && fr.height <= (1 << 20));
  int32_t q32 = -1;
  uint32_t work_px = 0;
  uint32_t ray_acc = 0;
  uint32_t pij = 0;
  int k = 0;
  bool has_px = false, done = false, active = false;
  bool heavy = false;
  V3 color = splat(0.f);
  V3 moment = splat(0.f);
  int k_end_px = 0;
  auto k_end = [&]() -> int {
    if constexpr (BUDGET) return k_end_px;
    else return fr.k_end;
  };
  auto feature_add3 = [&](float *buf, V3 v) {
    float *w = buf + (int64_t)q32 * 3;
    w[0] = __fadd_rn(w[0], v.x), w[1] = __fadd_rn(w[1], v.y), w[2] = __fadd_rn(w[2], v.z);
  };
  uint32_t rays = 0;
  Rng rng = {0, 0, 0, 0, 0, 0};
  V3 o = splat(0.f), d = splat(0.f);
  int depth = 0;
  const bool tex32 = (F & F_TEX) && (!QUEUE || tex_layers);
  auto tex_layer_offset = [&](int level) -> uint32_t {
    return (uint32_t)lc.stack_off + (((uint32_t)level * n_threads + threadIdx.x) << 2);
  };

  unsigned long long sparse_limit = 0ull;
  if ((F & F_BVH) && lc.sparse_items) sparse_limit = *lc.sparse_items;
  const bool classes = (F & F_BVH) && lc.head_list != nullptr && sparse_limit != 0ull;
  uint32_t end64 = 0u, end32 = 0u;
  if (classes) end64 = lc.sparse_items[1], end32 = lc.sparse_items[2];
  uint32_t thr64 = 0xffffffffu, thr32 = 0xffffffffu, thr16 = 0xffffffffu;
  if (classes && lc.exclusive && lc.promote) thr64 = lc.sparse_items[23], thr32 = lc.sparse_items[24], thr16 = lc.sparse_items[25];
  const bool promote = thr16 != 0xffffffffu;
  int cls = 1;
  bool head_open = classes;
  auto take_item = [&](int64_t item) -> bool {
    q32 = (int32_t)item;
    const int64_t q = item;
// ... 223 lines not shown
          const uint32_t nq = pool_at + rank;
          int64_t item = (int64_t)nq;
          if (lc.tile_order) item = (int64_t)lc.tile_order[nq >> 4] * 16 + (int64_t)(nq & 15u);
          (void)take_item(item);
        }
        pool_at += want_n < avail ? want_n : avail;
      }
    } else if (!active && !done) {
      while (!has_px && !done) {
        if ((F & F_BVH) && sparse_limit != 0ull && (threadIdx.x & (uint32_t)(lc.sparse_stride - 1)) != 0) {
          if (wave_heavy) break;
          if (__hip_atomic_load(&counters[0], __ATOMIC_RELAXED, __HIP_MEMORY_SCOPE_AGENT) < sparse_limit) break;
        }
        const unsigned long long nq = atomicAdd(&counters[0], 1ull);
        if ((int64_t)nq >= n_items) {
          done = true;
          break;
        }
        int64_t item = (int64_t)nq;
        if (lc.tile_order) item = (int64_t)lc.tile_order[nq >> 4] * 16 + (int64_t)(nq & 15);
        if (!take_item(item)) continue;
        heavy = nq < sparse_limit;
      }
    }
    if (!active && !done) {
      if (RAYS && has_px) {
        k++;
        depth = 0;
        active = true;
      } else if (has_px) {
        float r1 = rng_01(rng);
        float r2 = rng_01(rng);
        float xf, yf;
        if (f32_jitter) {
          xf = (r1 + (float)(pij & 0xffffu)) * (float)inv_w;
          yf = (r2 + (float)(fr.height - (int)(pij >> 16))) * (float)inv_h;
        } else {
          double x = (double)r1 + (double)(int)(pij & 0xffffu);
          double y = (double)r2 + (double)(fr.height - (int)(pij >> 16));
          x = w_pow2 ? x * inv_w : x / (double)fr.width;
          y = h_pow2 ? y * inv_h : y / (double)fr.height;
          x = 2 * x - 1;
          y = 2 * y - 1;
          x = (x + 1) / 2;
          y = (y + 1) / 2;
          xf = (float)x, yf = (float)y;
        }
        V3 target = sc.cam.llc + xf * sc.cam.horizontal + yf * sc.cam.vertical;
        V3 origin = sc.cam.position;
        if (F & F_DEFOCUS) {
          if (sc.cam.defocus) {
            float ox = rng_range(0.f, sc.cam.lens_radius, rng);
            float oy = rng_range(0.f, sc.cam.lens_radius, rng);
            origin = sc.cam.position + sc.cam.u * ox + sc.cam.v * oy;
          }
        }
        o = origin;
        d = unit3_rn_twice(target - origin);
        k++;
        if ((F & F_BVH) && promote && cls == 1 && k >= lc.promote) {
          const unsigned long long have = (unsigned long long)rays * (unsigned)lc.probe_spp, per = (unsigned long long)k;
          if (have >= thr16 * per) cls = have >= thr64 * per ? 64 : have >= thr32 * per ? 32 : 16;
        }
        depth = 0;
        active = true;
      }
    }
    if (!__any(active)) {
      if (!(F & F_BVH) || __all(done)) break;
      continue;
    }

#if defined(RTMI_STATS) && RTMI_STATS == 9
    if ((wave_queries + 1u) % 600u == 0u && (wave_queries + 1u) / 600u <= 9u && (threadIdx.x & 63u) == 0u)
      g_wave_stats[((blockIdx.x * blockDim.x + threadIdx.x) >> 6) & 16383u][(wave_queries + 1u) / 600u] =
          ((stat_real() - t_begin) & 0xffffffffffull) | ((unsigned long long)(st.node_steps + st.face_steps) << 40);
#endif
    RTMI_STAT(wave_queries++; const unsigned long long tq1 = stat_now(); st.cyc[0] += tq1 - tq0;
              const unsigned long long in0 = st.cyc[2] + st.cyc[3];)
    Hit h = {};
    const bool all_lanes_in = (F & F_BVH) || ((F & F_TRIS) && ((M & PIN_LDS_TABLES) || (ll != nullptr && sc.n_pairs >= kCullMinPairs))) ||
                              ((F & F_SGROUP) && cands != nullptr);
    if (all_lanes_in)
      h = closest_hit<F, false, M>(sc, s_nodes, lc.lds_nodes, s_paths, lc.lds_paths, s_pairs, ll, cands, wl, counters + (QUEUE ? 0 : 2), o, d, active,
                         (F & F_BVH) && lc.visit_counts != nullptr
#ifdef RTMI_STATS
                         , st
#endif
      );
    RTMI_STAT(const unsigned long long tq2 = stat_now(); st.cyc[1] += (tq2 - tq1) - (st.cyc[2] + st.cyc[3] - in0);)
#ifdef RTMI_CHECK_MARGINS
    if (!QUEUE && all_lanes_in && (check_tick++ % RTMI_CHECK_EVERY) == 0u) {
      const Hit h2 = closest_hit<F>(sc, s_nodes, 0, s_paths, 0, nullptr, nullptr, nullptr, nullptr, nullptr, o, d, active, false
#ifdef RTMI_STATS
                                    , st
#endif
      );
      const bool differs = active && (h2.ok != h.ok || (h.ok && (__float_as_uint(h2.t) != __float_as_uint(h.t) || h2.win != h.win ||
                                                                 ((F & F_BVH) && h2.aux != h.aux))));
      const unsigned long long na = __builtin_amdgcn_ballot_w64(active), nd = __builtin_amdgcn_ballot_w64(differs);
      if ((threadIdx.x & 63u) == 0u) {
        atomicAdd(&counters[33], (unsigned long long)__popcll(na));
        if (nd) atomicAdd(&counters[34], (unsigned long long)__popcll(nd));
      }
    }
#endif
    if (active) {
      if (!all_lanes_in)
        h = closest_hit<F, false, M & ~(uint32_t)PIN_LDS_TABLES>(sc, s_nodes, 0, s_paths, 0, s_pairs, nullptr, nullptr, nullptr, nullptr, o, d, true, false
#ifdef RTMI_STATS
                           , st
#endif
        );
      rays++;
      if ((F & F_BVH) && lc.visit_counts != nullptr) work_px += (uint32_t)h.work;

      V3 result = splat(0.f);
      bool ended = true;
      if (h.ok && depth < fr.max_depth) {
        const uint32_t kind = h.win >> 29;
        const uint32_t index = h.win & ID_INDEX_MASK;
        V3 p = o + h.t * d;
        if (kind == RUN_SKY) {
          V3 dir = unit3_rn(p);
          float tg = (float)(0.5 * ((double)dir.y + 1.0));
          float w0 = 1.0f - tg;
          result = mk(w0 * 1.0f + tg * 0.5f, w0 * 1.0f + tg * 0.7f, w0 * 1.0f + tg * 1.0f);
          if constexpr (FEATURES) {
            if (depth == 0 && feat->albedo) feature_add3(feat->albedo, result);
          }
        } else {
          V3 nrm = splat(0.f);
          int mat = 0;
          float tu = 0.f, tv = 0.f;
          if ((F & F_TRIS) && kind == RUN_TRIS) {
            V3 n;
            int flags;
            if ((M & PIN_LDS_TABLES) || s_pairs != nullptr) {
              const float4 tn = s_nrm[index];
              n = mk(tn.x, tn.y, tn.z);
              mat = __float_as_int(tn.w) & 0xffffff, flags = __float_as_int(tn.w) >> 24;
            } else {
              const HotTri &tr = sc.tris[index];
              n = mk(tr.n[0], tr.n[1], tr.n[2]);
              mat = tr.mat, flags = tr.flags;
            }
            nrm = dot3(d, n) < 0.f ? n : -n;
            if (F & F_TEX) {
              if (flags & TRI_PGRAM) {
                float w = (float)((1.0 - (double)h.u) - (double)h.v);
                if (!(flags & TRI_SECOND)) {
                  tu = (0.f * w + 1.f * h.u) + 0.f * h.v;
                  tv = (1.f * w + 1.f * h.u) + 0.f * h.v;
                } else {
                  tu = (1.f * w + 0.f * h.u) + 1.f * h.v;
                  tv = (1.f * w + 0.f * h.u) + 0.f * h.v;
                }
              } else {
                tu = h.u, tv = h.v;
              }
            }
          }
          if ((F & F_SPHERE) && kind == RUN_SPHERE) {
            const SphereRec &sr = sc.spheres[index];
            nrm = unit3_rn(p - mk(sr.cx, sr.cy, sr.cz));
            mat = sr.mat;
            if (F & F_TEX) {
              const float pi_f = 3.14159265358979323846264338327950288f;
              float theta = acosf(-nrm.y);
              float phi = atan2f(-nrm.z, nrm.x) + pi_f;
              tu = phi / (2 * pi_f);
              tv = theta / pi_f;
            }
          }
          if ((F & F_BVH) && kind == RUN_BVH) {
            const FaceRec &fc = sc.faces[index];
            V3 n = unit3_rn(cross3(mk(fc.e1[0], fc.e1[1], fc.e1[2]), mk(fc.e2[0], fc.e2[1], fc.e2[2])));
            nrm = dot3(d, n) < 0.f ? n : -n;
            const BvhRec br = sc.bvhs[h.aux];
            mat = br.mat;
            if ((F & F_TEX) && br.has_uv) {
              const float *tc = sc.face_uv + (size_t)(br.face_base + fc.orig) * 6;
              float w = (float)((1.0 - (double)h.u) - (double)h.v);
              tu = (tc[0] * w + tc[2] * h.u) + tc[4] * h.v;
              tv = (tc[1] * w + tc[3] * h.u) + tc[5] * h.v;
            }
          }
          MatRec m;
          {
            float4 m0;
            float2 m1;
            if (mats_in_lds) {
              m0 = load_lds<float4>(s_mats + mat), m1 = load_lds<float2>(reinterpret_cast<const char *>(s_mats + mat) + 16);
            } else {
              m0 = load_global<float4>(sc.mats + mat), m1 = load_global<float2>(reinterpret_cast<const char *>(sc.mats + mat) + 16);
            }
            m.r = m0.x, m.g = m0.y, m.b = m0.z, m.kind = __float_as_int(m0.w), m.param = m1.x, m.tex = __float_as_int(m1.y);
          }
          V3 rgb = mk(m.r, m.g, m.b);
          RTMI_STAT2(if (!(F & F_BVH)) { const unsigned long long tsa = stat_now();
            if ((int)(threadIdx.x & 63u) == __builtin_ctzll(__ballot(1))) g_wave_stats[((blockIdx.x * blockDim.x + threadIdx.x) >> 6) & 16383u][9] += tsa - tq2; })
          uint32_t layer = (uint32_t)mat;
          if (F & F_TEX) {
            if (m.tex >= 0 && (m.kind == MAT_LAMBERTIAN || m.kind == MAT_LIGHT)) {
              const uint32_t px = tex_fetch(sc.texs[m.tex], tu, (float)(1.0 - (double)tv));
              layer = 0x80000000u | px;
              if (m.kind == MAT_LIGHT) rgb = texel_rgb(px);
            }
          }
          if constexpr (FEATURES) {
            if (depth == 0) {
              if (feat->albedo) feature_add3(feat->albedo, ((F & F_TEX) && (layer >> 31)) ? texel_rgb(layer) : rgb);
              if (feat->normal) feature_add3(feat->normal, nrm);
              if (feat->depth) feat->depth[q32] = __fadd_rn(feat->depth[q32], h.t);
              if (feat->coverage) feat->coverage[q32] += 1u;
            }
          }
          if (m.kind == MAT_LIGHT) {
            result = rgb;
          } else {
            const float dn = dot3(d, nrm);
// ... 76 lines not shown
            for (; i >= 1; i -= 2, at -= step) {
              const uint32_t b0 = lds_byte(at);
              const int m0 = b0 >> 4, m1 = b0 & 15;
              { const V3 a_ = lds_rgb(m0); result = mk(a_.x * result.x, a_.y * result.y, a_.z * result.z); }
              { const V3 a_ = lds_rgb(m1); result = mk(a_.x * result.x, a_.y * result.y, a_.z * result.z); }
            }
          } else {
            uint32_t at = ids_offset(i >= 0 ? i : 0);
            for (; i >= 3; i -= 4, at -= 4u * step) {
              const int m0 = lds_byte(at), m1 = lds_byte(at - step), m2 = lds_byte(at - 2u * step), m3 = lds_byte(at - 3u * step);
              const V3 a0 = lds_rgb(m0), a1 = lds_rgb(m1);
              const V3 a2 = lds_rgb(m2), a3 = lds_rgb(m3);
              result = mk(a0.x * result.x, a0.y * result.y, a0.z * result.z);
              result = mk(a1.x * result.x, a1.y * result.y, a1.z * result.z);
              result = mk(a2.x * result.x, a2.y * result.y, a2.z * result.z);
              result = mk(a3.x * result.x, a3.y * result.y, a3.z * result.z);
            }
            for (; i >= 0; i--, at -= step) {
              const int m0 = lds_byte(at);
              { const V3 a_ = lds_rgb(m0); result = mk(a_.x * result.x, a_.y * result.y, a_.z * result.z); }
            }
          }
        }
        for (; !FOLD4 && i >= 0; i--) {
          V3 a;
          if (tex32) {
            const uint32_t lw = *reinterpret_cast<const uint32_t *>(smem + tex_layer_offset(i));
            if (lw >> 31) {
              a = texel_rgb(lw);
            } else if (mats_in_lds) {
              a = lds_rgb((int)lw);
            } else {
              a = mk(sc.mats[lw].r, sc.mats[lw].g, sc.mats[lw].b);
            }
          } else {
            const int mi = nibble_ids     ? (int)((smem[ids_offset(i >> 1)] >> ((i & 1) * 4)) & 15u)
                           : lc.wide_ids ? (int)*reinterpret_cast<const uint16_t *>(smem + ids_offset(i))
                                         : (int)smem[ids_offset(i)];
            if (mats_in_lds) {
              a = lds_rgb(mi);
            } else {
              a = mk(sc.mats[mi].r, sc.mats[mi].g, sc.mats[mi].b);
            }
          }
          if (sc.unsigned_colours) {
            result = mk(a.x * result.x, a.y * result.y, a.z * result.z);
          } else {
            result = mk(0.f + a.x * result.x, 0.f + a.y * result.y, 0.f + a.z * result.z);
          }
        }
        color = color + result;
        if constexpr (BUDGET)
          moment = mk(__fadd_rn(moment.x, __fmul_rn(result.x, result.x)), __fadd_rn(moment.y, __fmul_rn(result.y, result.y)),
                      __fadd_rn(moment.z, __fmul_rn(result.z, result.z)));
        active = false;
      }
    }
    RTMI_STAT(st.cyc[4] += stat_now() - tq2;)
  }

  if (RTMI_PRIO) wave_priority_leave(lc.prio_tab);
#undef RTMI_CHAINS
#undef RTMI_PRIO
  {
    unsigned long long ray_total = ray_acc;
    for (int off = 32; off > 0; off >>= 1) ray_total += __shfl_down(ray_total, off);
    if ((threadIdx.x & 63) == 0 && ray_total) atomicAdd(&counters[1], ray_total);
  }
#ifdef RTMI_STATS
  if (!QUEUE && (threadIdx.x & 63) == 0) {
    const unsigned v[13] = {wave_queries, st.searches, st.node_steps, st.face_steps, st.nodes_popped, st.blocks_popped,
                            st.insert_rounds, st.steps_hist[0], st.steps_hist[1], st.steps_hist[2], st.steps_hist[3],
                            st.steps_hist[4], st.steps_hist[5]};
    for (int i = 0; i < 13; i++) atomicAdd(&counters[4 + i], (unsigned long long)v[i]);
    for (int i = 0; i < 9; i++) atomicAdd(&counters[17 + i], st.cyc[i]);
    const unsigned long long life = stat_real() - t_begin;
    atomicAdd(&counters[26], life);
    atomicMax(&counters[27], life);
    atomicAdd(&counters[28], 1ull);
    atomicAdd(&counters[29], st.calib);
    atomicAdd(&counters[30], st.cull_bits);
    atomicAdd(&counters[31], st.cull_iters);
    atomicAdd(&counters[32], st.cull_rays);
    const unsigned wid = (blockIdx.x * blockDim.x + threadIdx.x) >> 6;
    if (!(F & F_BVH) && wid < 16384u) {
      atomicAdd(&counters[25], g_wave_stats[wid][9]);
      atomicAdd(&counters[6], g_wave_stats[wid][10]);
      g_wave_stats[wid][9] = 0, g_wave_stats[wid][10] = 0;
      g_wave_stats[wid][0] = life, g_wave_stats[wid][11] = wave_queries;
      g_wave_stats[wid][12] = t_begin_rt, g_wave_stats[wid][13] = __builtin_amdgcn_s_memrealtime();
      g_wave_stats[wid][14] = (unsigned long long)__builtin_amdgcn_s_getreg(0xF804) | ((unsigned long long)__builtin_amdgcn_s_getreg(0xF814) << 32);
    } else if (wid < 16384u) {
      g_wave_stats[wid][0] = life;
#if RTMI_STATS != 9
      for (int i = 0; i < 9; i++) g_wave_stats[wid][1 + i] = st.cyc[i];
#endif
      g_wave_stats[wid][10] = wave_queries, g_wave_stats[wid][11] = st.node_steps, g_wave_stats[wid][12] = st.face_steps;
      g_wave_stats[wid][13] = st.nodes_popped, g_wave_stats[wid][14] = st.insert_rounds;
      g_wave_stats[wid][15] = (st.cyc[9] << 32) | (st.cyc[10] >> 8);
    }
  }
#endif
}
```

### ray-tracing-cuda_amd/csrc/scene.h

```cpp
#pragma once
#include <stdint.h>

#include <string>
#include <vector>

#include "scene_dev.h"
#include "vec.h"

namespace rtmi {

struct HostTex {
  bool image = false;
  V3 rgb{0, 0, 0};
  std::vector<uint8_t> rgba;
  int h = 0, w = 0;
};

struct HostMat {
  int32_t kind = MAT_LAMBERTIAN;
  V3 rgb{0, 0, 0};
  float param = 0.f;
  int tex = -1;
};

enum ObjKind { OBJ_SPHERE, OBJ_TRI, OBJ_PGRAM, OBJ_BOX, OBJ_SKY, OBJ_BVH };

struct HostObj {
  ObjKind kind;
  int mat = -1;
  V3 p[18];
  double radius = 0;
  int bvh = -1;
};

struct HostBvh {
  std::vector<float> faces;
  std::vector<float> uvs;
  int n = 0, mat = -1, leaf_max = 2048;
};

struct Scene {
  std::vector<HostTex> texs;
  std::vector<HostMat> mats;
  std::vector<HostObj> world;
  std::vector<int> list_counts{0};
  std::vector<HostBvh> bvhs;
  CameraDev cam{};
  V3 cam_w{0, 0, 0};
  bool has_camera = false;

  bool committed = false;
  uint32_t features = 0;
  std::vector<Run> runs;
  std::vector<SphereRec> spheres;
  std::vector<HotTri> tris;
  std::vector<PairBox> pair_boxes;
  std::vector<PairPts> pair_pts;
  std::vector<TriNrm> tri_nrm;
  std::vector<SphGroup> sph_groups;
  std::vector<SphMember> sph_members;
  float sph_mag = 0.f;
  int64_t sliver_faces = 0;
  float list_mag = 0.f;
  int n_pgrams = 0, n_triangles = 0, n_spheres = 0;
  std::vector<BvhRec> bvh_recs;
  std::vector<BvhNode> nodes;
  std::vector<QNode4> qnodes;
  std::vector<BvhNode> tops;
  std::vector<int32_t> leaf_paths;
  int sub_depth = 0;
  std::vector<FaceRec> faces;
  std::vector<float> face_uv;
  std::vector<int32_t> face_of_orig;
  std::vector<MatRec> mat_recs;
  std::vector<TexRec> tex_recs;
  std::vector<int32_t> q_sphere_entry, q_pair_entry, q_bvh_entry, q_face_input;
  int32_t q_sky_entry = -1;
  std::vector<void *> dev_allocs;
  SceneDev dev{};
  QueryDev qdev{};
  unsigned long long *d_counters = nullptr;
  int device = -1;
  int64_t bytes_per_ray = 0;
  void *d_sched = nullptr;
  size_t sched_bytes = 0;

  std::string flatten();
  std::string check_margins() const;
};

TriRec make_tri(V3 p0, V3 p1, V3 p2);
void camera_pinhole(Scene &s, V3 pos, V3 look_at, V3 up, double fov, double aspect);
void camera_defocus(Scene &s, V3 pos, V3 look_at, V3 up, double fov, double aspect, double aperture, double focus);
void camera_raw(Scene &s, V3 pos, V3 llc, V3 horiz, V3 vert);
void box_from_points(const V3 p[4], V3 out[8]);
void box_faces(const V3 corners[8], V3 faces[18]);

}
```

### ray-tracing-cuda_amd/csrc/scene.hip

```cpp
#include "scene.h"

#include <algorithm>
#include <cmath>
#include <cstring>
#include <numeric>

namespace rtmi {

TriRec make_tri(V3 p0, V3 p1, V3 p2) {
  V3 e1 = p1 - p0, e2 = p2 - p0;
  V3 n = unit3(cross3(e1, e2));
  TriRec r;
  r.p0[0] = p0.x, r.p0[1] = p0.y, r.p0[2] = p0.z;
  r.e1[0] = e1.x, r.e1[1] = e1.y, r.e1[2] = e1.z;
  r.e2[0] = e2.x, r.e2[1] = e2.y, r.e2[2] = e2.z;
  r.n[0] = n.x, r.n[1] = n.y, r.n[2] = n.z;
  return r;
}

static HotTri hot_tri(V3 p0, V3 p1, V3 p2, int mat, int flags) {
  TriRec t = make_tri(p0, p1, p2);
  HotTri h{};
  for (int c = 0; c < 3; c++) h.p0[c] = t.p0[c], h.e1[c] = t.e1[c], h.e2[c] = t.e2[c], h.n[c] = t.n[c];
  h.mat = mat;
  h.flags = flags;
  return h;
}

static int face_slack_exponent(const V3 p[3]);

static void push_pair(Scene &s, const V3 *p, int n, int flags) {
  PairPts pp{};
  const V3 q[4] = {p[0], p[1], p[2], n == 4 ? p[3] : p[2]};
  for (int c = 0; c < 3; c++) {
    const float x[4] = {c == 0 ? q[0].x : c == 1 ? q[0].y : q[0].z, c == 0 ? q[1].x : c == 1 ? q[1].y : q[1].z,
                        c == 0 ? q[2].x : c == 1 ? q[2].y : q[2].z, c == 0 ? q[3].x : c == 1 ? q[3].y : q[3].z};
    pp.p0[c] = x[0], pp.p1[c] = x[1], pp.p2[c] = x[2], pp.p3[c] = x[3];
  }
  pp.flags = flags;
  PairBox bx{};
  float diag = 0.f, mag = 0.f;
  for (int c = 0; c < 3; c++) {
    const float x[4] = {pp.p0[c], pp.p1[c], pp.p2[c], pp.p3[c]};
    bx.mn[c] = fminf(fminf(x[0], x[1]), fminf(x[2], x[3]));
    bx.mx[c] = fmaxf(fmaxf(x[0], x[1]), fmaxf(x[2], x[3]));
    diag = fmaxf(diag, bx.mx[c] - bx.mn[c]);
    mag = fmaxf(mag, fmaxf(fabsf(bx.mn[c]), fabsf(bx.mx[c])));
  }
  const float pad = fixed_pad(diag, mag);
  for (int c = 0; c < 3; c++) bx.mn[c] -= pad, bx.mx[c] += pad;
  const V3 second[3] = {q[1], q[2], q[3]};
  if (face_slack_exponent(q) > 0 || (n == 4 && face_slack_exponent(second) > 0))
    for (int c = 0; c < 3; c++) bx.mn[c] = -INFINITY, bx.mx[c] = INFINITY;
  s.list_mag = fmaxf(s.list_mag, mag);
  s.pair_pts.push_back(pp);
  s.pair_boxes.push_back(bx);
}

static void push_pgram(Scene &s, V3 p0, V3 p1, V3 p2, int mat) {
  std::vector<HotTri> &out = s.tris;
  V3 p3 = p1 + p2 - p0;
  const HotTri first = hot_tri(p0, p1, p2, mat, TRI_PGRAM);
  HotTri second = hot_tri(p1, p2, p3, mat, TRI_PGRAM | TRI_SECOND);
  if (memcmp(first.e2, second.e2, sizeof(first.e2)) == 0) second.flags |= TRI_SAME_E2;
  out.push_back(first);
  out.push_back(second);
  const V3 q[4] = {p0, p1, p2, p3};
  push_pair(s, q, 4, PAIR_SECOND | ((second.flags & TRI_SAME_E2) ? PAIR_SAME_E2 : 0));
}

void box_from_points(const V3 p[4], V3 out[8]) {
  auto fourth = [](V3 a, V3 b, V3 c) { return c + b - a; };
  V3 q[4];
  q[3] = fourth(p[0], p[1], p[2]);
  q[2] = fourth(p[0], p[1], p[3]);
  q[1] = fourth(p[0], p[2], p[3]);
  q[0] = fourth(p[1], q[2], q[3]);
  for (int i = 0; i < 4; i++) out[i] = p[i], out[4 + i] = q[i];
}

void box_faces(const V3 corners[8], V3 faces[18]) {
  int k = 0;
  for (int set = 0; set < 2; set++) {
    const V3 *c = corners + set * 4;
    for (int i = 1; i <= 3; i++) {
      int x = i, y = (i + 1 == 4) ? 1 : x + 1;
      faces[k++] = c[0];
      faces[k++] = c[x];
      faces[k++] = c[y];
    }
  }
}

void camera_pinhole(Scene &s, V3 pos, V3 look_at, V3 up, double fov, double aspect) {
  CameraDev &c = s.cam;
  c.defocus = 0;
  c.lens_radius = -1.f;
  c.position = pos;
  V3 w = unit3(pos - look_at);
  c.u = unit3(cross3(up, w));
  c.v = unit3(cross3(w, c.u));
  double half_height = std::tan(fov / 2);
  double half_width = aspect * half_height;
  c.horizontal = c.u * static_cast<float>(2 * half_width);
  c.vertical = c.v * static_cast<float>(2 * half_height);
  c.llc = pos - w - c.u * static_cast<float>(half_width) - c.v * static_cast<float>(half_height);
  s.cam_w = w;
  s.has_camera = true;
}

void camera_defocus(Scene &s, V3 pos, V3 look_at, V3 up, double fov, double aspect, double aperture, double focus) {
  CameraDev &c = s.cam;
  c.defocus = 1;
  c.position = pos;
  V3 w = unit3(pos - look_at);
  c.u = unit3(cross3(up, w));
  c.v = unit3(cross3(w, c.u));
  double half_height = focus * std::tan(fov / 2);
  double half_width = aspect * half_height;
  c.horizontal = c.u * static_cast<float>(2 * half_width);
  c.vertical = c.v * static_cast<float>(2 * half_height);
  c.llc = pos - w - c.u * static_cast<float>(half_width) - c.v * static_cast<float>(half_height);
  c.lens_radius = (float)(aperture / 2);
  s.cam_w = w;
  s.has_camera = true;
}

void camera_raw(Scene &s, V3 pos, V3 llc, V3 horiz, V3 vert) {
  CameraDev &c = s.cam;
  c.defocus = 0;
  c.lens_radius = -1.f;
  c.position = pos;
  c.llc = llc;
  c.horizontal = horiz;
  c.vertical = vert;
  c.u = splat(0.f);
  c.v = splat(0.f);
  s.cam_w = splat(0.f);
  s.has_camera = true;
}

struct FacePts {
  V3 p[3];
  float uv[6];
  int orig;
  int input;
  uint32_t code;
  int leaf;
  int kexp;
};

// ... 261 lines not shown
      for (int a = 0; a < 3; a++) t.mn[a] = 1.f, t.mx[a] = -1.f;
      t.left = -1;
      t.right = 0;
    }
    tops.push_back(t);
  }
}

static std::string check_search_tree(const std::vector<QNode4> &qn, const std::vector<FacePts> &fp, int node, float mn[3],
                                     float mx[3], int *kexp) {
  const QNode4 &nd = qn[(size_t)node];
  for (int a = 0; a < 3; a++) mn[a] = INFINITY, mx[a] = -INFINITY;
  *kexp = 0;
  for (int c = 0; c < 4; c++) {
    if (nd.child[c] == -1) continue;
    float cmn[3] = {INFINITY, INFINITY, INFINITY}, cmx[3] = {-INFINITY, -INFINITY, -INFINITY};
    int ck = 0;
    if (nd.child[c] >= 0) {
      const std::string e = check_search_tree(qn, fp, nd.child[c], cmn, cmx, &ck);
      if (!e.empty()) return e;
    } else {
      const int enc = -(nd.child[c] + 1), cnt = enc & 7, first = enc >> 3;
      for (int i = first; i < first + cnt; i++) {
        ck = std::max(ck, fp[(size_t)i].kexp);
        for (int j = 0; j < 3; j++) {
          const float q[3] = {fp[(size_t)i].p[j].x, fp[(size_t)i].p[j].y, fp[(size_t)i].p[j].z};
          for (int a = 0; a < 3; a++) cmn[a] = fminf(cmn[a], q[a]), cmx[a] = fmaxf(cmx[a], q[a]);
        }
      }
    }
    float diag = 0.f, mag = 0.f;
    for (int a = 0; a < 3; a++) diag = fmaxf(diag, cmx[a] - cmn[a]), mag = fmaxf(mag, fmaxf(fabsf(cmn[a]), fabsf(cmx[a])));
    const float pad = fixed_pad(diag, mag);
    for (int a = 0; a < 3; a++) {
      const double lo = (double)nd.origin[a] + std::ldexp((double)nd.qlo[a][c], nd.exp[a]);
      const double hi = (double)nd.origin[a] + std::ldexp((double)nd.qhi[a][c], nd.exp[a]);
      if (!(lo <= (double)cmn[a] - 0.98 * (double)pad && hi >= (double)cmx[a] + 0.98 * (double)pad))
        return "margin budget: a search node's child box does not contain its faces' padded bounds";
    }
    if (nd.slack_exp < ck) return "margin budget: a search node's slack exponent is below a face's under it";
    for (int a = 0; a < 3; a++) mn[a] = fminf(mn[a], cmn[a]), mx[a] = fmaxf(mx[a], cmx[a]);
    *kexp = std::max(*kexp, ck);
  }
  return "";
}

static int build_bvh_nodes(std::vector<BvhNode> &nodes, std::vector<FacePts> &fp, int first, int n, int leaf_max,
                           int level, uint32_t code, int *ref_depth, std::vector<int> &path,
                           std::vector<std::vector<int>> &leaf_paths) {
  if (level > *ref_depth) *ref_depth = level;
  BvhNode nd;
  for (int k = 0; k < 3; k++) nd.mn[k] = INFINITY, nd.mx[k] = -INFINITY;
  for (int i = 0; i < n; i++)
    for (int j = 0; j < 3; j++) {
      const V3 &p = fp[first + i].p[j];
      const float c[3] = {p.x, p.y, p.z};
      for (int k = 0; k < 3; k++) {
        nd.mn[k] = fminf(c[k], nd.mn[k]);
        nd.mx[k] = fmaxf(c[k], nd.mx[k]);
      }
    }
  int me = (int)nodes.size();
  nodes.push_back(nd);
  if (level > 0) path.push_back(me);
  if (n <= leaf_max) {
    nodes[me].left = -1;
    nodes[me].right = -n;
    for (int i = 0; i < n; i++) fp[first + i].code = code, fp[first + i].leaf = (int)leaf_paths.size();
    leaf_paths.push_back(path);
  } else {
    int mid = (n - 1) / 2;
    const uint32_t bit = level < 32 ? 0x80000000u >> level : 0u;
    int l = build_bvh_nodes(nodes, fp, first, mid + 1, leaf_max, level + 1, code, ref_depth, path, leaf_paths);
    int r = build_bvh_nodes(nodes, fp, first + mid + 1, n - mid - 1, leaf_max, level + 1, code | bit, ref_depth, path,
                            leaf_paths);
    nodes[me].left = l;
    nodes[me].right = r;
  }
  if (level > 0) path.pop_back();
  return me;
}

std::string Scene::flatten() {
  pair_boxes.clear(), pair_pts.clear(), tri_nrm.clear(), list_mag = 0.f;
  sph_groups.clear(), sph_members.clear(), sph_mag = 0.f;
  sliver_faces = 0;
  runs.clear(), spheres.clear(), tris.clear(), bvh_recs.clear(), face_of_orig.clear(), nodes.clear(), qnodes.clear(), faces.clear(), leaf_paths.clear(), tops.clear(),
      face_uv.clear(), mat_recs.clear(), tex_recs.clear();
  q_sphere_entry.clear(), q_pair_entry.clear(), q_bvh_entry.clear(), q_face_input.clear(), q_sky_entry = -1;
  features = 0;
  n_pgrams = n_triangles = n_spheres = 0;
  sub_depth = 0;
  if (!has_camera) return "scene has no camera";
  if (list_counts.empty() || list_counts[0] > 1024) return "world exceeds HitableList::kMaxHitables (1024)";
  if (cam.defocus) features |= F_DEFOCUS;

  std::vector<int> tex_to_image(texs.size(), -1);
  int n_images = 0;
  for (size_t i = 0; i < texs.size(); i++)
    if (texs[i].image) tex_to_image[i] = n_images++;
  for (const HostMat &m : mats) {
    MatRec r{};
    r.kind = m.kind;
    r.r = m.rgb.x, r.g = m.rgb.y, r.b = m.rgb.z;
    r.param = m.param;
    r.tex = -1;
    if (m.tex >= 0) {
      if (m.tex >= (int)texs.size()) return "material refers to an unknown texture";
      const HostTex &t = texs[m.tex];
      if (t.image) {
        r.tex = tex_to_image[m.tex];
        features |= F_TEX;
      } else {
        r.r = t.rgb.x, r.g = t.rgb.y, r.b = t.rgb.z;
      }
    }
    mat_recs.push_back(r);
  }
  if (mats.size() > (size_t)kMaxStackMats) features |= F_TEX;

  auto push_run = [&](int kind, int first) {
    const int stride = kind == RUN_TRIS ? 2 : 1;
    if (!runs.empty() && runs.back().kind == kind && runs.back().first + stride * runs.back().count == first) {
      runs.back().count++;
    } else {
      runs.push_back(Run{kind, first, 1, -1});
    }
  };
  auto check_mat = [&](int m) { return m >= 0 && m < (int)mats.size(); };
  if (mats.size() > (size_t)kMaxMats) return "more than 2^24 materials (TriNrm::mat_flags)";

  bytes_per_ray = 32;
  for (const HostObj &ob : world) {
    const int32_t entry = (int32_t)(&ob - world.data());
    auto name_pairs = [&](int32_t kind) {
      for (int32_t face = 0; (size_t)(q_pair_entry.size() / 2) < tris.size() / 2; face++)
        q_pair_entry.push_back(entry), q_pair_entry.push_back(kind | face << 8);
    };
    switch (ob.kind) {
      case OBJ_SKY:
        if (q_sky_entry < 0) q_sky_entry = entry;
        runs.push_back(Run{RUN_SKY, 0, 1, 0});
        break;
      case OBJ_SPHERE: {
        if (!check_mat(ob.mat)) return "sphere without a valid material";
        SphereRec r;
        r.cx = ob.p[0].x, r.cy = ob.p[0].y, r.cz = ob.p[0].z;
        r.mat = ob.mat;
        r.radius = ob.radius;
        r.r2 = ob.radius * ob.radius;
        spheres.push_back(r);
        q_sphere_entry.push_back(entry);
        push_run(RUN_SPHERE, (int)spheres.size() - 1);
        features |= F_SPHERE;
        bytes_per_ray += 28;
        break;
      }
      case OBJ_TRI: {
        if (!check_mat(ob.mat)) return "triangle without a valid material";
        tris.push_back(hot_tri(ob.p[0], ob.p[1], ob.p[2], ob.mat, 0));
        tris.push_back(HotTri{});
        push_pair(*this, ob.p, 3, 0);
        push_run(RUN_TRIS, (int)tris.size() - 2);
        name_pairs(QHIT_TRIANGLE);
        features |= F_TRIS;
        n_triangles++;
        bytes_per_ray += 40;
        break;
      }
      case OBJ_PGRAM: {
        if (!check_mat(ob.mat)) return "parallelogram without a valid material";
        push_pgram(*this, ob.p[0], ob.p[1], ob.p[2], ob.mat);
        push_run(RUN_TRIS, (int)tris.size() - 2);
        name_pairs(QHIT_PARALLELOGRAM);
        features |= F_TRIS;
        n_pgrams++;
        bytes_per_ray += 40;
        break;
      }
      case OBJ_BOX: {
        if (!check_mat(ob.mat)) return "parallelepiped without a valid material";
        for (int fidx = 0; fidx < 6; fidx++) {
          push_pgram(*this, ob.p[fidx * 3], ob.p[fidx * 3 + 1], ob.p[fidx * 3 + 2], ob.mat);
          push_run(RUN_TRIS, (int)tris.size() - 2);
          n_pgrams++;
          bytes_per_ray += 40;
        }
        name_pairs(QHIT_PARALLELEPIPED);
        features |= F_TRIS;
        break;
      }
      case OBJ_BVH: {
        const HostBvh &hb = bvhs[ob.bvh];
        if (hb.mat >= (int)mats.size()) return "bvh refers to an unknown material";
        if (hb.mat < 0) return "bvh without a material (material_ptr_ == nullptr) is not renderable";
        const bool has_uv = !hb.uvs.empty();
        std::vector<FacePts> fp((size_t)hb.n);
        for (int i = 0; i < hb.n; i++) {
          for (int j = 0; j < 3; j++)
            fp[i].p[j] = mk(hb.faces[(size_t)i * 9 + j * 3], hb.faces[(size_t)i * 9 + j * 3 + 1],
                            hb.faces[(size_t)i * 9 + j * 3 + 2]);
          for (int j = 0; j < 6; j++) fp[i].uv[j] = has_uv ? hb.uvs[(size_t)i * 6 + j] : 0.f;
          fp[i].kexp = face_slack_exponent(fp[i].p);
          fp[i].input = i;
          if (fp[i].kexp > 0) sliver_faces++;
        }
        int leaf_max = hb.leaf_max > 0 ? hb.leaf_max : 2048;
        if (hb.n > leaf_max)
          std::stable_sort(fp.begin(), fp.end(),
                           [](const FacePts &a, const FacePts &b) { return a.p[0].x < b.p[0].x; });
        for (int i = 0; i < hb.n; i++) fp[i].orig = i;
        const int face_base = (int)faces.size();
        const int sub_base = (int)qnodes.size();
        BvhRec br{};
        std::vector<BvhNode> local_nodes;
        std::vector<QNode4> local_sub;
        int depth = 0;
        int ref_depth = 0;
        std::vector<int> path_now;
        std::vector<std::vector<int>> local_paths;
        br.root = hb.n > 0 ? build_bvh_nodes(local_nodes, fp, 0, hb.n, leaf_max, 0, 0u, &ref_depth, path_now, local_paths) : -1;
        if (ref_depth > kRefDepthMax) return "mesh tree too deep for the kernel's leaf path codes";
        br.sub_root = hb.n > 0 ? build_subtree(local_sub, fp, 0, hb.n, &depth) + sub_base : -1;
        sub_depth = std::max(sub_depth, depth);
        if (depth > kSubDepthMax) return "mesh too deep for the kernel's search stack";
        if (hb.n > 0) {
          float tmn[3], tmx[3];
          int tk = 0;
          const std::string e = check_search_tree(local_sub, fp, 0, tmn, tmx, &tk);
          if (!e.empty()) return e;
        }
        if ((int64_t)face_base + hb.n + 4 >= kMeshMaxFaces || (int64_t)sub_base + (int64_t)local_sub.size() >= kMeshMaxNodes)
          return "mesh too large for the kernel's 26-bit search-stack entries";
        const int node_base = (int)nodes.size();
        for (BvhNode nd : local_nodes) {
          if (nd.right >= 0) nd.left += node_base, nd.right += node_base;
          nodes.push_back(nd);
        }
        for (QNode4 nd : local_sub) {
          for (int c = 0; c < 4; c++) {
            if (nd.child[c] >= 0) {
              nd.child[c] += sub_base;
            } else {
              const int enc = -(nd.child[c] + 1), cnt = enc & 7, first = enc >> 3;
              nd.child[c] = cnt ? -((first + face_base) * 8 + cnt) - 1 : -1;
// ... 75 lines not shown
      const SphereRec &sp = spheres[run.first + i];
      const double c[3] = {sp.cx, sp.cy, sp.cz};
      uint32_t code = 0;
      for (int a = 0; a < 3; a++) {
        const double ext = hi[a] - lo[a];
        uint32_t qv = ext > 0 ? (uint32_t)std::min(1023.0, std::floor((c[a] - lo[a]) / ext * 1024.0)) : 0u;
        for (int bit = 0; bit < 10; bit++) code |= ((qv >> bit) & 1u) << (3 * bit + a);
      }
      if (std::fabs(sp.radius) > big) code |= 0x80000000u;
      order[i] = {code, i};
    }
    std::stable_sort(order.begin(), order.end());
    run.pad = (int)sph_groups.size();
    for (int g0 = 0; g0 < run.count; g0 += kSphGroupSize) {
      SphGroup g{};
      g.first = (int)sph_members.size();
      g.count = std::min(kSphGroupSize, run.count - g0);
      float mn[3] = {INFINITY, INFINITY, INFINITY}, mx[3] = {-INFINITY, -INFINITY, -INFINITY};
      for (int k = 0; k < g.count; k++) {
        const int idx = run.first + order[g0 + k].second;
        const SphereRec &sp = spheres[idx];
        SphMember m{};
        m.cx = sp.cx, m.cy = sp.cy, m.cz = sp.cz, m.r2f = (float)sp.r2, m.orig = idx, m.r2 = sp.r2;
        sph_members.push_back(m);
        const float r = (float)(std::fabs(sp.radius) * (1.0 + (double)kSphRadiusPad)) + kPadFloor;
        const float c[3] = {sp.cx, sp.cy, sp.cz};
        for (int a = 0; a < 3; a++) mn[a] = fminf(mn[a], c[a] - r), mx[a] = fmaxf(mx[a], c[a] + r);
      }
      float diag = 0.f, mag = 0.f;
      for (int a = 0; a < 3; a++) diag = fmaxf(diag, mx[a] - mn[a]), mag = fmaxf(mag, fmaxf(fabsf(mn[a]), fabsf(mx[a])));
      const float pad = fixed_pad(diag, mag) + kSphDistSlack * mag;
      for (int a = 0; a < 3; a++) g.mn[a] = mn[a] - pad, g.mx[a] = mx[a] + pad;
      sph_mag = fmaxf(sph_mag, mag);
      sph_groups.push_back(g);
    }
  }
  if (!sph_groups.empty()) features |= F_SGROUP;
  if (!sph_groups.empty()) {
    sph_groups.push_back(SphGroup{});
    sph_members.push_back(SphMember{});
  }
  for (size_t t = 0; t < 2 * pair_pts.size() && t < tris.size(); t++) {
    TriNrm r{};
    for (int c = 0; c < 3; c++) r.n[c] = tris[t].n[c];
    r.mat_flags = (tris[t].mat & 0xffffff) | (tris[t].flags << 24);
    tri_nrm.push_back(r);
  }
  if (!tris.empty()) {
    tris.push_back(HotTri{});
    tris.push_back(HotTri{});
    pair_boxes.push_back(PairBox{});
  }
  n_spheres = (int)spheres.size();
  if (!spheres.empty()) spheres.push_back(SphereRec{});
  for (const MatRec &m : mat_recs)
    if (m.tex >= 0) bytes_per_ray += 4;
  return check_margins();
}

std::string Scene::check_margins() const {
  for (size_t i = 0; i < pair_pts.size(); i++) {
    const PairPts &pp = pair_pts[i];
    const PairBox &bx = pair_boxes[i];
    const bool lone = !(tris[2 * i].flags & TRI_PGRAM);
    const V3 q[4] = {mk(pp.p0[0], pp.p0[1], pp.p0[2]), mk(pp.p1[0], pp.p1[1], pp.p1[2]), mk(pp.p2[0], pp.p2[1], pp.p2[2]),
                     lone ? mk(pp.p2[0], pp.p2[1], pp.p2[2]) : mk(pp.p3[0], pp.p3[1], pp.p3[2])};
    const V3 second[3] = {q[1], q[2], q[3]};
    const bool thin = face_slack_exponent(q) > 0 || (!lone && face_slack_exponent(second) > 0);
    float mn[3] = {INFINITY, INFINITY, INFINITY}, mx[3] = {-INFINITY, -INFINITY, -INFINITY};
    for (int j = 0; j < 4; j++) {
      const float c[3] = {q[j].x, q[j].y, q[j].z};
      for (int a = 0; a < 3; a++) mn[a] = fminf(mn[a], c[a]), mx[a] = fmaxf(mx[a], c[a]);
    }
    float diag = 0.f, mag = 0.f;
    for (int a = 0; a < 3; a++) diag = fmaxf(diag, mx[a] - mn[a]), mag = fmaxf(mag, fmaxf(fabsf(mn[a]), fabsf(mx[a])));
    const double pad = 0.98 * (double)fixed_pad(diag, mag);
    for (int a = 0; a < 3; a++) {
      if (thin ? !(bx.mn[a] == -INFINITY && bx.mx[a] == INFINITY)
               : !((double)bx.mn[a] <= (double)mn[a] - pad && (double)bx.mx[a] >= (double)mx[a] + pad))
        return "margin budget: a world-list pair's bounds do not cover what its triangle tests can accept";
    }
    if (!(mag <= list_mag)) return "margin budget: list_mag is below a pair's coordinates";
  }
  for (size_t g = 0; g + 1 < sph_groups.size(); g++) {
    const SphGroup &gr = sph_groups[g];
    float mn[3] = {INFINITY, INFINITY, INFINITY}, mx[3] = {-INFINITY, -INFINITY, -INFINITY};
    for (int k = 0; k < gr.count; k++) {
      const SphMember &m = sph_members[(size_t)gr.first + k];
      const double r = std::fabs(spheres[(size_t)m.orig].radius) * (1.0 + (double)kSphRadiusPad) * 0.999999;
      const float c[3] = {m.cx, m.cy, m.cz};
      for (int a = 0; a < 3; a++) mn[a] = fminf(mn[a], (float)((double)c[a] - r)), mx[a] = fmaxf(mx[a], (float)((double)c[a] + r));
    }
    float diag = 0.f, mag = 0.f;
    for (int a = 0; a < 3; a++) diag = fmaxf(diag, mx[a] - mn[a]), mag = fmaxf(mag, fmaxf(fabsf(mn[a]), fabsf(mx[a])));
    const double pad = 0.98 * ((double)fixed_pad(diag, mag) + (double)kSphDistSlack * mag);
    for (int a = 0; a < 3; a++)
      if (!((double)gr.mn[a] <= (double)mn[a] - pad && (double)gr.mx[a] >= (double)mx[a] + pad))
        return "margin budget: a sphere group's bounds do not cover what its members' pre-tests can accept";
  }
  for (size_t b = 0; b < bvh_recs.size(); b++) {
    const size_t n_lo = (size_t)bvh_recs[b].sub_root;
    const size_t n_hi = b + 1 < bvh_recs.size() ? (size_t)bvh_recs[b + 1].sub_root : qnodes.size();
    for (int i = 0; i < kTopEntries; i++) {
      const BvhNode &t = tops[b * kTopEntries + (size_t)i];
      if (t.left == -1) continue;
      bool found = false;
      for (size_t n = n_lo; n < n_hi && !found; n++)
        for (int c = 0; c < 4 && !found; c++)
          if (qnodes[n].child[c] == t.left) {
            found = true;
            for (int a = 0; a < 3; a++) {
              const double lo = (double)qnodes[n].origin[a] + std::ldexp((double)qnodes[n].qlo[a][c], qnodes[n].exp[a]);
              const double hi = (double)qnodes[n].origin[a] + std::ldexp((double)qnodes[n].qhi[a][c], qnodes[n].exp[a]);
              if (!((double)t.mn[a] <= lo && (double)t.mx[a] >= hi)) return "margin budget: a top-table entry is smaller than the child box it stands for";
            }
            if (t.right < qnodes[n].slack_exp) return "margin budget: a top-table entry's slack exponent is below its node's";
          }
      if (!found) return "margin budget: a top-table entry refers to no child of the search tree";
    }
  }
  return "";
}


}
```

### ray-tracing-cuda_amd/csrc/scene_dev.h

```cpp
#pragma once
#include <stdint.h>

#include "vec.h"
#include "margins.h"

namespace rtmi {

enum RunKind : int32_t { RUN_SKY = 0, RUN_SPHERE = 1, RUN_TRIS = 2, RUN_BVH = 4 };

struct Run {
  int32_t kind, first, count, pad;
};

struct SphereRec {
  float cx, cy, cz;
  int32_t mat;
  double radius;
  double r2;
};

struct SphGroup {
  float mn[3], mx[3];
  int32_t first, count;
};
struct SphMember {
  float cx, cy, cz;
  float r2f;
  int32_t orig;
  int32_t pad;
  double r2;
};
constexpr int kSphGroupSize = 16;
constexpr int kSphGroupMin = 32;
constexpr int kSphCand = 16;

struct TriRec {
  float p0[3];
  float e1[3];
  float e2[3];
  float n[3];
};

enum : int32_t { TRI_SECOND = 1, TRI_PGRAM = 2, TRI_SAME_E2 = 4 };
struct HotTri {
  float p0[3];
  float e1[3];
  float e2[3];
  float n[3];
  int32_t mat;
  int32_t flags;
  int32_t pad[2];
};

enum : int32_t { PAIR_SECOND = 1, PAIR_SAME_E2 = 2 };
struct PairBox {
  float mn[3], mx[3];
  int32_t pad[2];
};
struct alignas(16) PairPts {
  float p0[3], p1[3], p2[3], p3[3];
  int32_t flags;
  int32_t pad[3];
};
struct alignas(16) TriNrm {
  float n[3];
  int32_t mat_flags;
};
constexpr int kMaxStackMats = 1 << 16;
constexpr int kMaxMats = 1 << 24;
constexpr int kCullMinPairs = 4;
constexpr int kListTasks(uint32_t features) { return (features & 16u) ? 96 : (features & 4u) ? 128 : 192; }
constexpr int kListWaveWords(uint32_t features) {
  return 64 * 8 + kListTasks(features) * (1 + ((features & 16u) ? 6 : (features & 1u) ? 3 : 2));
}
constexpr int kLdsPairs = 128;

enum MatKind : int32_t { MAT_LAMBERTIAN = 0, MAT_METAL = 1, MAT_DIELECTRIC = 2, MAT_LIGHT = 3, MAT_SKY = 4 };

struct alignas(16) MatRec {
  float r, g, b;
  int32_t kind;
  float param;
  int32_t tex;
  int32_t pad[2];
};

struct TexRec {
  const uint8_t *rgba;
  int32_t height, width;
  int64_t pitch;
  int64_t pad;
};

struct BvhNode {
  float mn[3];
  float mx[3];
  int32_t left;
  int32_t right;
};

struct alignas(16) QNode4 {
  float origin[3];
  int8_t exp[3];
  int8_t slack_exp;
  uint8_t qlo[3][4];
  uint8_t qhi[3][4];
  uint32_t pad1[2];
  int32_t child[4];
};
constexpr int kSlackExpMax = 24;
constexpr int kSubDepthMax = 80;
constexpr int kMeshFaceSlack = 68;
constexpr int kHitSlots = 4;
constexpr int kHitWords = 3;
constexpr int kMeshRayWords = 16 + kHitSlots * kHitWords;
constexpr int kMeshStackWords = 512;
constexpr int kMeshWaveWords = 64 * kMeshRayWords + kMeshStackWords;
constexpr uint32_t kCodeNone = 0xffffffffu;
constexpr int kSparseStride = 16;
constexpr int kTopEntries = 64;
constexpr int kTopRays = 16;
constexpr int kLeafPathMax = 1 << 26;
constexpr int kLdsPaths = 1024;
constexpr int kRefDepthMax = 31;
constexpr int kMeshMaxFaces = 1 << 23;
constexpr int kMeshMaxNodes = 1 << 26;

struct BvhRec {
  int32_t root;
  int32_t mat;
  int32_t has_uv;
  int32_t face_base;
  int32_t sub_root;
  float mag;
  int32_t ref_depth;
  int32_t path_base;
  float root_mn[3], root_mx[3];
  int32_t n_faces;
  int32_t slack_exp;
};
static_assert(sizeof(BvhRec) == 64, "BvhRec is read with one s_load_dwordx16");

struct alignas(16) FaceRec {
  float p0[3];
  float e1[3];
  float e2[3];
  int32_t orig;
  uint32_t code;
  int32_t leaf;
};

struct CameraDev {
  V3 position, llc, horizontal, vertical, u, v;
  float lens_radius;
  int32_t defocus;
};

constexpr int kPrioRows = 1 << 14;
constexpr size_t kPrioTabBytes = (size_t)kPrioRows * 16 * sizeof(uint32_t);

constexpr int kLdsMats = 512;
constexpr int kLdsNodes = 512;

struct SceneDev {
  const Run *runs;
  const SphereRec *spheres;
  const HotTri *tris;
  const PairBox *pair_boxes;
  const SphGroup *sph_groups;
  const SphMember *sph_members;
  float sph_mag;
  int32_t n_sph_groups;
  const PairPts *pair_pts;
  const TriNrm *tri_nrm;
  const BvhRec *bvhs;
  const BvhNode *nodes;
  const QNode4 *qnodes;
  const BvhNode *tops;
  const int32_t *leaf_paths;
  int32_t n_leaf_paths;
  const FaceRec *faces;
  const float *face_uv;
#ifdef RTMI_CHECK_MARGINS
  const int32_t *face_of_orig;
#endif
  const MatRec *mats;
  const TexRec *texs;
  int32_t n_runs, n_mats, n_nodes;
  int32_t n_pairs;
  float list_mag;
  int32_t sub_reserve;
  int32_t det_safe;
  int32_t unsigned_colours;
  CameraDev cam;
};

enum : int32_t { QHIT_NONE = 0, QHIT_SPHERE = 1, QHIT_TRIANGLE = 2, QHIT_PARALLELOGRAM = 3, QHIT_PARALLELEPIPED = 4,
                 QHIT_MESH = 5, QHIT_SKY = 6 };
struct QueryDev {
  const int32_t *sphere_entry;
  const int32_t *pair_entry;
  const int32_t *bvh_entry;
  const int32_t *face_input;
  int32_t sky_entry;
};

enum : uint32_t {
  F_SPHERE = 1u,
  F_TRIS = 2u,
  F_SGROUP = 4u,
  F_BVH = 8u,
  F_TEX = 16u,
  F_DEFOCUS = 32u,
  F_ALL = 63u
};

struct FrameDev {
  int32_t height, width, spp, max_depth, post;
  int32_t k_begin, k_end;
  int32_t rank, world;
  int32_t tiles_x, tiles_y, n_tiles;
  int32_t local_tiles;
  int64_t items;
};

struct FeatureBufs {
  float *albedo = nullptr;
  float *normal = nullptr;
  float *depth = nullptr;
  uint32_t *coverage = nullptr;
};

}
```

### ray-tracing-cuda_amd/rtmi/__init__.py

```python
import collections
import ctypes as C
import os

import numpy as np

_PKG_DIR = os.path.dirname(os.path.abspath(__file__))
_ROOT = os.path.dirname(_PKG_DIR)
LIB_PATH = os.environ.get("RTMI_LIB_PATH") or os.path.join(_ROOT, "lib", "librtmi.so")

TILE = 8
STATE_WORDS = 6
MAX_DEPTH = 64
TRACE_WORK_WORDS = 256
BUDGET_WORK_WORDS = TRACE_WORK_WORDS
MODE_FIELDS = 9
FAST_PATH_FACTS = 14
MAX_MATERIALS = 1 << 24

RTMI_HIT_NONE = 0
RTMI_HIT_SPHERE = 1
RTMI_HIT_TRIANGLE = 2
RTMI_HIT_PARALLELOGRAM = 3
RTMI_HIT_PARALLELEPIPED = 4
RTMI_HIT_MESH = 5
# ... 453 lines not shown
        _check(self.L.rtmi_add_sphere(self.h, _f(c)[1], float(r), mat), "rtmi_add_sphere")

    def triangle(self, p, mat):
        _check(self.L.rtmi_add_triangle(self.h, _f(p)[1], mat), "rtmi_add_triangle")

    def parallelogram(self, p, mat):
        _check(self.L.rtmi_add_parallelogram(self.h, _f(p)[1], mat), "rtmi_add_parallelogram")

    def parallelepiped(self, p, mat):
        _check(self.L.rtmi_add_parallelepiped(self.h, _f(p)[1], mat), "rtmi_add_parallelepiped")

    def parallelepiped_lengths(self, lengths, mat, transform):
        def cb(pin, pout, _user):
            o = transform(np.array([pin[0], pin[1], pin[2]], dtype=np.float32))
            pout[0], pout[1], pout[2] = float(o[0]), float(o[1]), float(o[2])

        cfn = TRANSFORM_FN(cb)
        self._keep.append(cfn)
        _check(self.L.rtmi_add_parallelepiped_lengths(self.h, _f(lengths)[1], mat, cfn, None),
               "rtmi_add_parallelepiped_lengths")

    def sky(self):
        _check(self.L.rtmi_add_sky(self.h), "rtmi_add_sky")

    def list_begin(self):
        _check(self.L.rtmi_list_begin(self.h), "rtmi_list_begin")

    def list_end(self):
        _check(self.L.rtmi_list_end(self.h), "rtmi_list_end")

    def bvh(self, faces, mat, uvs=None, k_min=2048):
        faces = np.ascontiguousarray(faces, dtype=np.float32).reshape(-1, 9)
        uvp = None
        if uvs is not None:
            uvs = np.ascontiguousarray(uvs, dtype=np.float32).reshape(-1, 6)
            uvp = uvs.ctypes.data_as(_fp)
        _check(self.L.rtmi_add_bvh(self.h, faces.ctypes.data_as(_fp), uvp, faces.shape[0],
                                   -1 if mat is None else mat, k_min), "rtmi_add_bvh")

    def camera_pinhole(self, pos, look_at, up, fov, aspect):
        _check(self.L.rtmi_camera_pinhole(self.h, _f(pos)[1], _f(look_at)[1], _f(up)[1], float(fov), float(aspect)),
               "rtmi_camera_pinhole")

    def camera_defocus(self, pos, look_at, up, fov, aspect, aperture, focus):
        _check(self.L.rtmi_camera_defocus(self.h, _f(pos)[1], _f(look_at)[1], _f(up)[1], float(fov), float(aspect),
                                          float(aperture), float(focus)), "rtmi_camera_defocus")

    def camera_raw(self, pos, llc, horiz, vert):
        _check(self.L.rtmi_camera_raw(self.h, _f(pos)[1], _f(llc)[1], _f(horiz)[1], _f(vert)[1]), "rtmi_camera_raw")

    def camera_get(self):
        out = np.zeros(21, dtype=np.float32)
        _check(self.L.rtmi_camera_get(self.h, out.ctypes.data_as(_fp)), "rtmi_camera_get")
        return out.reshape(7, 3)

    def camera_update(self, frame21, defocus=False, lens_radius=-1.0):
        f = _camera21(frame21, "frame21")
        _check(self.L.rtmi_camera_update(self.h, f.ctypes.data_as(_fp), 1 if defocus else 0, float(lens_radius)),
               "rtmi_camera_update")
        return self

    def camera_look(self, pos, look_at, up, fov, aspect):
        tmp = C.c_void_p(self.L.rtmi_scene_create())
        try:
            _check(self.L.rtmi_camera_pinhole(tmp, _f(pos)[1], _f(look_at)[1], _f(up)[1], float(fov), float(aspect)),
                   "rtmi_camera_pinhole")
            f = np.zeros(21, dtype=np.float32)
            _check(self.L.rtmi_camera_get(tmp, f.ctypes.data_as(_fp)), "rtmi_camera_get")
        finally:
            self.L.rtmi_scene_destroy(tmp)
        return self.camera_update(f)

    def random_float(self, mn, mx):
        return np.float32(self.L.rtmi_rng_host_random_float(C.c_float(float(np.float32(mn))),
                                                            C.c_float(float(np.float32(mx))),
                                                            self.state0.ctypes.data_as(_u32p)))

    def stats(self):
        out = (C.c_int64 * 8)()
        _check(self.L.rtmi_scene_stats(self.h, out), "rtmi_scene_stats")
        keys = ["world", "spheres", "parallelograms", "triangles", "bvh_faces", "bvh_nodes", "materials", "textures"]
        return dict(zip(keys, list(out)))

    def sliver_faces(self):
        return _check(self.L.rtmi_scene_sliver_faces(self.h), "rtmi_scene_sliver_faces")

    def bytes_per_ray(self):
        return _check(self.L.rtmi_scene_bytes_per_ray(self.h), "rtmi_scene_bytes_per_ray")

    def commit(self):
        _check(self.L.rtmi_scene_commit(self.h), "rtmi_scene_commit")
        self.device = None
        try:
            import torch
            if torch.cuda.is_available():
                self.device = torch.device("cuda", torch.cuda.current_device())
        except ImportError:
            pass
        return self

    def intersect(self, origins, directions, t_max=None, out=None):
        import torch
        n, dev, t_max = _check_batch("rtmi_intersect", origins, directions, t_max)
        out = _out_buffer(out, "int32 tensor of shape (N, 12)", (n, HIT_WORDS), dev, torch.int32)
        stream = self._stream(dev)
        origins, directions = origins.contiguous(), directions.contiguous()
        abandoned = torch.zeros((1,), dtype=torch.int64, device=dev)
        with torch.cuda.device(dev):
            _check(self.L.rtmi_intersect(self.h, n, C.c_void_p(origins.data_ptr()), C.c_void_p(directions.data_ptr()),
                                         C.c_void_p(t_max.data_ptr()) if t_max is not None else None,
                                         C.c_void_p(out.data_ptr()), C.c_void_p(abandoned.data_ptr()), stream),
                   "rtmi_intersect")
        f = out.view(torch.float32)
        hits = Hits(f[:, 0], f[:, 1:3], f[:, 3:6], out[:, 6], out[:, 7], out[:, 8], out[:, 9])
        hits.raw, hits.abandoned = out, abandoned
        hits._rays = (origins, directions, t_max)
        return hits

    def occluded(self, origins, directions, t_max=None, out=None):
        import torch
        n, dev, t_max = _check_batch("rtmi_occluded", origins, directions, t_max)
        out = _out_buffer(out, "uint8 or bool tensor of shape (N,)", (n,), dev, torch.uint8, torch.bool)
        stream = self._stream(dev)
        origins, directions = origins.contiguous(), directions.contiguous()
        raw = out.view(torch.uint8)
        counts = torch.zeros((2,), dtype=torch.int64, device=dev)
        with torch.cuda.device(dev):
            _check(self.L.rtmi_occluded(self.h, n, C.c_void_p(origins.data_ptr()), C.c_void_p(directions.data_ptr()),
                                        C.c_void_p(t_max.data_ptr()) if t_max is not None else None,
                                        C.c_void_p(raw.data_ptr()), C.c_void_p(counts.data_ptr()), stream),
                   "rtmi_occluded")
        return Occlusion(raw, counts, (origins, directions, t_max))

    def trace(self, origins, directions, states, max_depth, count_rays=False, out=None):
        import torch
        n, dev, _ = _check_batch("rtmi_trace", origins, directions)
        if not _is_buffer(states, (STATE_WORDS, n), dev, torch.int32):
            raise RtmiError("states must be a contiguous CUDA int32 tensor of shape (6, N) on the rays' device")
        max_depth = int(max_depth)
        if not 0 <= max_depth <= MAX_DEPTH:
            raise RtmiError("max_depth %d outside [0, %d]" % (max_depth, MAX_DEPTH))
        out = _out_buffer(out, "float32 tensor of shape (N, 3)", (n, 3), dev, torch.float32)
        stream = self._stream(dev)
        origins, directions = origins.contiguous(), directions.contiguous()
        rays = torch.empty((n,), dtype=torch.int32, device=dev) if count_rays else None
        work = torch.zeros((TRACE_WORK_WORDS,), dtype=torch.int64, device=dev)
        with torch.cuda.device(dev):
            _check(self.L.rtmi_trace(self.h, n, C.c_void_p(origins.data_ptr()), C.c_void_p(directions.data_ptr()),
                                     max_depth, C.c_void_p(states.data_ptr()), C.c_void_p(out.data_ptr()),
                                     C.c_void_p(rays.data_ptr()) if rays is not None else None,
                                     C.c_void_p(work.data_ptr()), stream), "rtmi_trace")
        return Trace(out, rays, work, (origins, directions, states))

    def _stream(self, dev):
        if self.h.value is None or getattr(self, "device", None) is None:
            raise RtmiError("scene not committed")
        if dev != self.device:
            raise RtmiError("the rays are on %s, the scene was committed on %s" % (dev, self.device))
        import torch
        return C.c_void_p(torch.cuda.current_stream(dev).cuda_stream)


def _check_batch(entry, origins, directions, t_max=None):
    try:
        import torch
    except ImportError:
# ... 276 lines not shown
```

Measured before the change: 32660.

## Store list triangles as precomputed base-point/edge records instead of pair corners

Replaces the 64-byte four-corner pair records with two 48-byte per-triangle records that hold the base point and precomputed edges. This removes the edge subtractions in the hot intersection loop and lets the batched task loop spread one triangle per lane instead of one pair per lane. In exchange, the LDS footprint per pair and the staging copy grow from 16 to 24 words, which may lower occupancy or push scenes out of the LDS path. The global fallback reads the HotTri records, and the device upload of tri_pts only happens when the pairs fit in LDS. It also adds debug entry points and a histogram stat.

```diff
diff --git a/ray-tracing-cuda_amd/csrc/capi.hip b/ray-tracing-cuda_amd/csrc/capi.hip
--- a/ray-tracing-cuda_amd/csrc/capi.hip
+++ b/ray-tracing-cuda_amd/csrc/capi.hip
@@ -438,7 +438,7 @@
   if ((rc = upload(s, s->spheres, &d.spheres))) return rc;
   if ((rc = upload(s, s->tris, &d.tris))) return rc;
   if ((rc = upload(s, s->pair_boxes, &d.pair_boxes))) return rc;
-  if ((rc = upload(s, s->pair_pts, &d.pair_pts))) return rc;
+  if ((int)s->pair_pts.size() <= kLdsPairs && (rc = upload(s, s->tri_pts, &d.tri_pts))) return rc;
   if ((rc = upload(s, s->tri_nrm, &d.tri_nrm))) return rc;
   if ((rc = upload(s, s->sph_groups, &d.sph_groups))) return rc;
   if ((rc = upload(s, s->sph_members, &d.sph_members))) return rc;
@@ -530,6 +530,31 @@
   Scene tmp;
   if (int rc = flattened(sp, &tmp)) return rc;
   return tmp.bytes_per_ray;
+}
+
+int64_t rtmi_debug_list_records(const rtmi_scene *sp, int64_t cap_pairs, uint32_t *tri_pts, uint32_t *hot_tris, float *corners) {
+  if (!sp) return fail(RTMI_ERR_INVALID, "null scene");
+  Scene tmp;
+  if (int rc = flattened(sp, &tmp)) return rc;
+  const int64_t n = (int64_t)tmp.pair_pts.size();
+  for (int64_t i = 0; i < n && i < cap_pairs; i++) {
+    if (tri_pts) memcpy(tri_pts + 24 * i, &tmp.tri_pts[2 * i], 2 * sizeof(TriPts));
+    if (hot_tris) memcpy(hot_tris + 32 * i, &tmp.tris[2 * i], 2 * sizeof(HotTri));
+    if (corners) memcpy(corners + 12 * i, tmp.pair_pts[i].p0, 12 * sizeof(float));
+  }
+  return n;
+}
+
+int64_t rtmi_debug_render_lds_bytes(const rtmi_scene *sp, int max_depth, int threads) {
+  if (!sp || max_depth < 0 || threads < 64 || threads % 64) return fail(RTMI_ERR_INVALID, "bad arguments");
+  Scene tmp;
+  if (int rc = flattened(sp, &tmp)) return rc;
+  SceneDev d{};
+  d.n_pairs = (int)tmp.pair_pts.size(), d.n_mats = (int)tmp.mat_recs.size(), d.n_nodes = (int)tmp.nodes.size();
+  d.n_leaf_paths = (int)tmp.leaf_paths.size(), d.n_sph_groups = (int)tmp.sph_groups.size();
+  FrameDev fr{};
+  fr.max_depth = max_depth;
+  return (int64_t)render_lds_bytes(pick_variant(tmp.features), d, fr, threads);
 }
 
 int64_t rtmi_frame_work_items(const rtmi_frame *f) {
diff --git a/ray-tracing-cuda_amd/csrc/closest_hit.h b/ray-tracing-cuda_amd/csrc/closest_hit.h
--- a/ray-tracing-cuda_amd/csrc/closest_hit.h
+++ b/ray-tracing-cuda_amd/csrc/closest_hit.h
@@ -51,9 +51,27 @@
 }
 #endif
 
+template <uint32_t M>
+__device__ __forceinline__ bool load_tri_pts(const SceneDev &sc, const float4 *s_tris, int rec, int which, V3 &p0, V3 &e1, V3 &e2) {
+  float4 qa, qb, qc;
+  bool present;
+  if ((M & PIN_LDS_TABLES) || s_tris != nullptr) {
+    const float4 *pp = s_tris + (size_t)rec * 3;
+    qa = load_lds<float4>(pp), qb = load_lds<float4>(pp + 1), qc = load_lds<float4>(pp + 2);
+    present = !(__float_as_int(qc.y) & TRIPTS_ABSENT);
+  } else {
+    const float4 *pp = reinterpret_cast<const float4 *>(sc.tris + rec);
+    qa = load_global<float4>(pp), qb = load_global<float4>(pp + 1), qc = load_global<float4>(pp + 2);
+    const float4 qd = load_global<float4>(pp + 3);
+    present = which == 0 || (__float_as_int(qd.y) & TRI_SECOND);
+  }
+  p0 = mk(qa.x, qa.y, qa.z), e1 = mk(qa.w, qb.x, qb.y), e2 = mk(qb.z, qb.w, qc.x);
+  return present;
+}
+
 template <uint32_t F, bool OCC = false, uint32_t M = 0>
 __device__ __forceinline__ Hit closest_hit(const SceneDev &sc, const BvhNode *s_nodes, int lds_nodes, const int *s_paths,
-                                           int lds_paths, const float4 *s_pairs, int *ll, uint16_t *cands, int *wl,
+                                           int lds_paths, const float4 *s_tris, int *ll, uint16_t *cands, int *wl,
                                            unsigned long long *overflow, V3 o, V3 d, bool live, bool count_work
 #ifdef RTMI_STATS
                                            , MeshStats &st
@@ -159,24 +177,14 @@
           if (mask != 0u) {
             const int bit = __builtin_ctz(mask);
             mask &= mask - 1u;
-            const size_t pidx = (size_t)(pair0 + c0 + bit) * 4;
-            float4 qa, qb, qc, qd;
-            if ((M & PIN_LDS_TABLES) || s_pairs != nullptr) {
-              const float4 *pp = s_pairs + pidx;
-              qa = load_lds<float4>(pp), qb = load_lds<float4>(pp + 1), qc = load_lds<float4>(pp + 2), qd = load_lds<float4>(pp + 3);
-            } else {
-              const float4 *pp = reinterpret_cast<const float4 *>(sc.pair_pts) + pidx;
-              qa = load_global<float4>(pp), qb = load_global<float4>(pp + 1), qc = load_global<float4>(pp + 2), qd = load_global<float4>(pp + 3);
-            }
-            const V3 p0 = mk(qa.x, qa.y, qa.z), p1 = mk(qa.w, qb.x, qb.y), p2 = mk(qb.z, qb.w, qc.x), p3 = mk(qc.y, qc.z, qc.w);
+            const int rec = 2 * (pair0 + c0 + bit);
+            V3 p0, e1, e2, p1, e1b, e2b;
+            (void)load_tri_pts<M>(sc, s_tris, rec, 0, p0, e1, e2);
+            const bool second = load_tri_pts<M>(sc, s_tris, rec + 1, 1, p1, e1b, e2b);
             float ta = 0.f, ua = 0.f, va = 0.f, tb = 0.f, ub = 0.f, vb = 0.f;
-            const V3 e1 = p1 - p0, e2 = p2 - p0;
             const bool hit_a = tri_test_flat<T>(p0, e1, e2, cross3(d, e2), o, d, t_to, ta, ua, va, det_safe);
             bool hit_b = false;
-            if (__float_as_int(qd.x) & PAIR_SECOND) {
-              const V3 e1b = p2 - p1, e2b = p3 - p1;
-              hit_b = tri_test_flat<T>(p1, e1b, e2b, cross3(d, e2b), o, d, t_to, tb, ub, vb, det_safe) && !hit_a;
-            }
+            if (second) hit_b = tri_test_flat<T>(p1, e1b, e2b, cross3(d, e2b), o, d, t_to, tb, ub, vb, det_safe) && !hit_a;
             const float t = hit_a ? ta : tb;
             const bool acc = (hit_a || hit_b) && (!ok || (T)t < t_to);
             ok = ok || acc;
@@ -213,15 +221,16 @@
             const int lo_t = __builtin_amdgcn_readlane(base, __builtin_ctzll(__builtin_amdgcn_ballot_w64(todo)));
             const bool now = todo && base + cnt - lo_t <= kListTasks(F);
             const int n_now = __builtin_amdgcn_readlane(base + cnt, 63 - __builtin_clzll(__builtin_amdgcn_ballot_w64(now))) - lo_t;
+            RTMI_STAT(st.nnow_hist[(n_now - 1) >> 5 < 5 ? (n_now - 1) >> 5 : 5]++;)
             if (now) {
               int k = base - lo_t;
               for (uint32_t m = mask; m != 0u; m &= m - 1u) tasks[k++] = (lane << 5) | __builtin_ctz(m);
             }
             wave_lds_fence();
-            for (int t0 = 0; t0 < n_now; t0 += 64) {
+            for (int t0 = 0; t0 < 2 * n_now; t0 += 64) {
               const int ti = t0 + lane;
-              if (ti < n_now) {
-                const int w = tasks[ti];
+              if (ti < 2 * n_now) {
+                const int w = tasks[ti >> 1], which = ti & 1;
                 const int *orr = ll + (w >> 5) * 8;
                 const float4 r0 = *reinterpret_cast<const float4 *>(orr), r1 = *reinterpret_cast<const float4 *>(orr + 4);
                 T t0_to;
@@ -231,30 +240,14 @@
                   t0_to = (T)r0.w;
                 }
                 const V3 ro = mk(r0.x, r0.y, r0.z), rd = mk(r1.x, r1.y, r1.z);
-                const size_t pidx = (size_t)(pair0 + c0 + (w & 31)) * 4;
-                float4 qa, qb, qc, qd;
-                if ((M & PIN_LDS_TABLES) || s_pairs != nullptr) {
-                  const float4 *pp = s_pairs + pidx;
-                  qa = load_lds<float4>(pp), qb = load_lds<float4>(pp + 1), qc = load_lds<float4>(pp + 2), qd = load_lds<float4>(pp + 3);
-                } else {
-                  const float4 *pp = reinterpret_cast<const float4 *>(sc.pair_pts) + pidx;
-                  qa = load_global<float4>(pp), qb = load_global<float4>(pp + 1), qc = load_global<float4>(pp + 2), qd = load_global<float4>(pp + 3);
-                }
-                const V3 p0 = mk(qa.x, qa.y, qa.z), p1 = mk(qa.w, qb.x, qb.y), p2 = mk(qb.z, qb.w, qc.x), p3 = mk(qc.y, qc.z, qc.w);
-                float ta = 0.f, ua = 0.f, va = 0.f, tb = 0.f, ub = 0.f, vb = 0.f;
-                const V3 e1 = p1 - p0, e2 = p2 - p0;
-                const bool hit_a = tri_test_flat<T>(p0, e1, e2, cross3(rd, e2), ro, rd, t0_to, ta, ua, va, det_safe);
-                bool hit_b = false;
-                if (__float_as_int(qd.x) & PAIR_SECOND) {
-                  const V3 e1b = p2 - p1, e2b = p3 - p1;
-                  hit_b = tri_test_flat<T>(p1, e1b, e2b, cross3(rd, e2b), ro, rd, t0_to, tb, ub, vb, det_safe);
-                }
-                int *res = results + ti * RW;
-                res[0] = hit_a ? __float_as_int(ta) : (int)0xffffffff;
-                res[1] = hit_b ? __float_as_int(tb) : (int)0xffffffff;
-                if (F & F_TEX) {
-                  res[2] = __float_as_int(ua), res[3] = __float_as_int(va), res[4] = __float_as_int(ub), res[5] = __float_as_int(vb);
-                }
+                V3 p0, e1, e2;
+                const bool present = load_tri_pts<M>(sc, s_tris, 2 * (pair0 + c0 + (w & 31)) + which, which, p0, e1, e2);
+                float tt = 0.f, uu = 0.f, vv = 0.f;
+                bool hit = false;
+                if (present) hit = tri_test_flat<T>(p0, e1, e2, cross3(rd, e2), ro, rd, t0_to, tt, uu, vv, det_safe);
+                int *res = results + (ti >> 1) * RW;
+                res[which] = hit ? __float_as_int(tt) : (int)0xffffffff;
+                if (F & F_TEX) res[2 + 2 * which] = __float_as_int(uu), res[3 + 2 * which] = __float_as_int(vv);
               }
             }
             wave_lds_fence();
diff --git a/ray-tracing-cuda_amd/csrc/kernels.h b/ray-tracing-cuda_amd/csrc/kernels.h
--- a/ray-tracing-cuda_amd/csrc/kernels.h
+++ b/ray-tracing-cuda_amd/csrc/kernels.h
@@ -69,6 +69,7 @@
 };
 uint32_t fast_path_mode(const FastPathFacts &f);
 FastPathFacts fast_path_facts(uint32_t variant, const SceneDev &sc, const FrameDev &fr, int threads, int enabled);
+size_t render_lds_bytes(uint32_t variant, const SceneDev &sc, const FrameDev &fr, int threads);
 struct SchedPlan {
   const uint32_t *tile_order = nullptr;
   uint32_t *visit_counts = nullptr;
diff --git a/ray-tracing-cuda_amd/csrc/kernels.hip b/ray-tracing-cuda_amd/csrc/kernels.hip
--- a/ray-tracing-cuda_amd/csrc/kernels.hip
+++ b/ray-tracing-cuda_amd/csrc/kernels.hip
@@ -494,7 +494,7 @@
   const bool cull = (variant & F_TRIS) && sc.n_pairs >= kCullMinPairs && !plain_list_scan();
   const bool staged = cull && sc.n_pairs <= kLdsPairs;
   lc.pairs_off = staged ? (int32_t)poff : -1;
-  size_t noff2 = (poff + (staged ? (size_t)sc.n_pairs * sizeof(PairPts) : 0) + 15) & ~(size_t)15;
+  size_t noff2 = (poff + (staged ? (size_t)sc.n_pairs * 2 * sizeof(TriPts) : 0) + 15) & ~(size_t)15;
   lc.nrm_off = staged ? (int32_t)noff2 : -1;
   size_t loff = (noff2 + (staged ? (size_t)sc.n_pairs * 2 * sizeof(TriNrm) : 0) + 15) & ~(size_t)15;
   const bool groups = (variant & F_SGROUP) && sc.n_sph_groups > 0;
@@ -568,6 +568,12 @@
   f.pairs_in_lds = lc.pairs_off >= 0 && lc.nrm_off >= 0 && lc.list_off >= 0;
   f.unsigned_colours = sc.unsigned_colours, f.det_safe = sc.det_safe, f.width = fr.width, f.height = fr.height;
   return f;
+}
+
+size_t render_lds_bytes(uint32_t variant, const SceneDev &sc, const FrameDev &fr, int threads) {
+  size_t lds = 0;
+  (void)make_cfg(variant, sc, fr, threads, &lds);
+  return lds;
 }
 
 template <auto Kernel>
diff --git a/ray-tracing-cuda_amd/csrc/mesh_search.h b/ray-tracing-cuda_amd/csrc/mesh_search.h
--- a/ray-tracing-cuda_amd/csrc/mesh_search.h
+++ b/ray-tracing-cuda_amd/csrc/mesh_search.h
@@ -102,6 +102,7 @@
 struct MeshStats {
   unsigned searches, node_steps, face_steps, nodes_popped, blocks_popped, insert_rounds, steps_hist[6];
   unsigned long long cull_bits, cull_rays, cull_iters;
+  unsigned nnow_hist[6];
   unsigned long long calib;
   unsigned long long cyc[11];
 };
diff --git a/ray-tracing-cuda_amd/csrc/occlusion_body.h b/ray-tracing-cuda_amd/csrc/occlusion_body.h
--- a/ray-tracing-cuda_amd/csrc/occlusion_body.h
+++ b/ray-tracing-cuda_amd/csrc/occlusion_body.h
@@ -17,7 +17,7 @@
 struct QueryLds {
   const BvhNode *s_nodes;
   const int *s_paths;
-  const float4 *s_pairs;
+  const float4 *s_tris;
   int *wl, *ll;
   uint16_t *cands;
 };
@@ -28,12 +28,12 @@
   q.wl = nullptr;
   if (F & F_BVH)
     q.wl = reinterpret_cast<int *>(smem + lc.mesh_off) + __builtin_amdgcn_readfirstlane((int)(threadIdx.x >> 6)) * kMeshWaveWords;
-  q.s_pairs = nullptr;
+  q.s_tris = nullptr;
   if ((F & F_TRIS) && lc.pairs_off >= 0) {
-    q.s_pairs = reinterpret_cast<const float4 *>(smem + lc.pairs_off);
-    const uint32_t *src = reinterpret_cast<const uint32_t *>(sc.pair_pts);
+    q.s_tris = reinterpret_cast<const float4 *>(smem + lc.pairs_off);
+    const uint32_t *src = reinterpret_cast<const uint32_t *>(sc.tri_pts);
     uint32_t *dst = reinterpret_cast<uint32_t *>(smem + lc.pairs_off);
-    for (int w = threadIdx.x; w < sc.n_pairs * 16; w += blockDim.x) dst[w] = src[w];
+    for (int w = threadIdx.x; w < sc.n_pairs * 24; w += blockDim.x) dst[w] = src[w];
   }
   q.ll = nullptr;
   if ((F & (F_TRIS | F_SGROUP)) && lc.list_off >= 0)
@@ -125,14 +125,14 @@
       const double start = pass == 0 ? start0 : (double)INFINITY;
       Hit h = {};
       if (all_lanes_in)
-        h = closest_hit<F, true>(sc, q.s_nodes, lc.lds_nodes, q.s_paths, lc.lds_paths, q.s_pairs, q.ll, q.cands, q.wl,
+        h = closest_hit<F, true>(sc, q.s_nodes, lc.lds_nodes, q.s_paths, lc.lds_paths, q.s_tris, q.ll, q.cands, q.wl,
                                  counts, o, d, go, false
 #ifdef RTMI_STATS
                                  , st
 #endif
                                  , start, seed, &unc);
       else if (go)
-        h = closest_hit<F, true>(sc, q.s_nodes, 0, q.s_paths, 0, q.s_pairs, nullptr, nullptr, nullptr, nullptr, o, d, true,
+        h = closest_hit<F, true>(sc, q.s_nodes, 0, q.s_paths, 0, q.s_tris, nullptr, nullptr, nullptr, nullptr, o, d, true,
                                  false
 #ifdef RTMI_STATS
                                  , st
diff --git a/ray-tracing-cuda_amd/csrc/query_body.h b/ray-tracing-cuda_amd/csrc/query_body.h
--- a/ray-tracing-cuda_amd/csrc/query_body.h
+++ b/ray-tracing-cuda_amd/csrc/query_body.h
@@ -92,12 +92,12 @@
   int *wl = nullptr;
   if (F & F_BVH)
     wl = reinterpret_cast<int *>(smem + lc.mesh_off) + __builtin_amdgcn_readfirstlane((int)(threadIdx.x >> 6)) * kMeshWaveWords;
-  const float4 *s_pairs = nullptr;
+  const float4 *s_tris = nullptr;
   if ((F & F_TRIS) && lc.pairs_off >= 0) {
-    s_pairs = reinterpret_cast<const float4 *>(smem + lc.pairs_off);
-    const uint32_t *src = reinterpret_cast<const uint32_t *>(sc.pair_pts);
+    s_tris = reinterpret_cast<const float4 *>(smem + lc.pairs_off);
+    const uint32_t *src = reinterpret_cast<const uint32_t *>(sc.tri_pts);
     uint32_t *dst = reinterpret_cast<uint32_t *>(smem + lc.pairs_off);
-    for (int w = threadIdx.x; w < sc.n_pairs * 16; w += blockDim.x) dst[w] = src[w];
+    for (int w = threadIdx.x; w < sc.n_pairs * 24; w += blockDim.x) dst[w] = src[w];
   }
   int *ll = nullptr;
   if ((F & (F_TRIS | F_SGROUP)) && lc.list_off >= 0)
@@ -145,13 +145,13 @@
     }
     Hit h = {};
     if (all_lanes_in)
-      h = closest_hit<F>(sc, s_nodes, lc.lds_nodes, s_paths, lc.lds_paths, s_pairs, ll, cands, wl, abandoned, o, d, live, false
+      h = closest_hit<F>(sc, s_nodes, lc.lds_nodes, s_paths, lc.lds_paths, s_tris, ll, cands, wl, abandoned, o, d, live, false
 #ifdef RTMI_STATS
                          , st
 #endif
       );
     else if (live)
-      h = closest_hit<F>(sc, s_nodes, 0, s_paths, 0, s_pairs, nullptr, nullptr, nullptr, nullptr, o, d, true, false
+      h = closest_hit<F>(sc, s_nodes, 0, s_paths, 0, s_tris, nullptr, nullptr, nullptr, nullptr, o, d, true, false
 #ifdef RTMI_STATS
                          , st
 #endif
diff --git a/ray-tracing-cuda_amd/csrc/render_body.h b/ray-tracing-cuda_amd/csrc/render_body.h
--- a/ray-tracing-cuda_amd/csrc/render_body.h
+++ b/ray-tracing-cuda_amd/csrc/render_body.h
@@ -153,12 +153,12 @@
   if (F & F_BVH)
     wl = reinterpret_cast<int *>(smem + lc.mesh_off) +
          __builtin_amdgcn_readfirstlane((int)(threadIdx.x >> 6)) * kMeshWaveWords;
-  const float4 *s_pairs = nullptr;
+  const float4 *s_tris = nullptr;
   if ((F & F_TRIS) && ((M & PIN_LDS_TABLES) || lc.pairs_off >= 0)) {
-    s_pairs = reinterpret_cast<const float4 *>(smem + lc.pairs_off);
-    const uint32_t *src = reinterpret_cast<const uint32_t *>(sc.pair_pts);
+    s_tris = reinterpret_cast<const float4 *>(smem + lc.pairs_off);
+    const uint32_t *src = reinterpret_cast<const uint32_t *>(sc.tri_pts);
     uint32_t *dst = reinterpret_cast<uint32_t *>(smem + lc.pairs_off);
-    for (int w = threadIdx.x; w < sc.n_pairs * 16; w += blockDim.x) dst[w] = src[w];
+    for (int w = threadIdx.x; w < sc.n_pairs * 24; w += blockDim.x) dst[w] = src[w];
     const uint32_t *nsrc = reinterpret_cast<const uint32_t *>(sc.tri_nrm);
     uint32_t *ndst = reinterpret_cast<uint32_t *>(smem + lc.nrm_off);
     for (int w = threadIdx.x; w < sc.n_pairs * 8; w += blockDim.x) ndst[w] = nsrc[w];
@@ -548,7 +548,7 @@
     const bool all_lanes_in = (F & F_BVH) || ((F & F_TRIS) && ((M & PIN_LDS_TABLES) || (ll != nullptr && sc.n_pairs >= kCullMinPairs))) ||
                               ((F & F_SGROUP) && cands != nullptr);
     if (all_lanes_in)
-      h = closest_hit<F, false, M>(sc, s_nodes, lc.lds_nodes, s_paths, lc.lds_paths, s_pairs, ll, cands, wl, counters + (QUEUE ? 0 : 2), o, d, active,
+      h = closest_hit<F, false, M>(sc, s_nodes, lc.lds_nodes, s_paths, lc.lds_paths, s_tris, ll, cands, wl, counters + (QUEUE ? 0 : 2), o, d, active,
                          (F & F_BVH) && lc.visit_counts != nullptr
 #ifdef RTMI_STATS
                          , st
@@ -573,7 +573,7 @@
 #endif
     if (active) {
       if (!all_lanes_in)
-        h = closest_hit<F, false, M & ~(uint32_t)PIN_LDS_TABLES>(sc, s_nodes, 0, s_paths, 0, s_pairs, nullptr, nullptr, nullptr, nullptr, o, d, true, false
+        h = closest_hit<F, false, M & ~(uint32_t)PIN_LDS_TABLES>(sc, s_nodes, 0, s_paths, 0, s_tris, nullptr, nullptr, nullptr, nullptr, o, d, true, false
 #ifdef RTMI_STATS
                            , st
 #endif
@@ -602,7 +602,7 @@
           if ((F & F_TRIS) && kind == RUN_TRIS) {
             V3 n;
             int flags;
-            if ((M & PIN_LDS_TABLES) || s_pairs != nullptr) {
+            if ((M & PIN_LDS_TABLES) || s_tris != nullptr) {
               const float4 tn = s_nrm[index];
               n = mk(tn.x, tn.y, tn.z);
               mat = __float_as_int(tn.w) & 0xffffff, flags = __float_as_int(tn.w) >> 24;
@@ -845,6 +845,8 @@
     atomicAdd(&counters[30], st.cull_bits);
     atomicAdd(&counters[31], st.cull_iters);
     atomicAdd(&counters[32], st.cull_rays);
+    for (int i = 0; i < 3; i++)
+      atomicAdd(&counters[37 + i], (unsigned long long)st.nnow_hist[2 * i] | ((unsigned long long)st.nnow_hist[2 * i + 1] << 32));
     const unsigned wid = (blockIdx.x * blockDim.x + threadIdx.x) >> 6;
     if (!(F & F_BVH) && wid < 16384u) {
       atomicAdd(&counters[25], g_wave_stats[wid][9]);
diff --git a/ray-tracing-cuda_amd/csrc/scene.h b/ray-tracing-cuda_amd/csrc/scene.h
--- a/ray-tracing-cuda_amd/csrc/scene.h
+++ b/ray-tracing-cuda_amd/csrc/scene.h
@@ -39,6 +39,10 @@
   int n = 0, mat = -1, leaf_max = 2048;
 };
 
+struct PairPts {
+  float p0[3], p1[3], p2[3], p3[3];
+};
+
 struct Scene {
   std::vector<HostTex> texs;
   std::vector<HostMat> mats;
@@ -56,6 +60,7 @@
   std::vector<HotTri> tris;
   std::vector<PairBox> pair_boxes;
   std::vector<PairPts> pair_pts;
+  std::vector<TriPts> tri_pts;
   std::vector<TriNrm> tri_nrm;
   std::vector<SphGroup> sph_groups;
   std::vector<SphMember> sph_members;
diff --git a/ray-tracing-cuda_amd/csrc/scene.hip b/ray-tracing-cuda_amd/csrc/scene.hip
--- a/ray-tracing-cuda_amd/csrc/scene.hip
+++ b/ray-tracing-cuda_amd/csrc/scene.hip
@@ -29,7 +29,25 @@
 
 static int face_slack_exponent(const V3 p[3]);
 
-static void push_pair(Scene &s, const V3 *p, int n, int flags) {
+static TriPts tri_pts(V3 a, V3 b, V3 c, int flags) {
+  const V3 e1 = b - a, e2 = c - a;
+  TriPts r{};
+  r.p0[0] = a.x, r.p0[1] = a.y, r.p0[2] = a.z;
+  r.e1[0] = e1.x, r.e1[1] = e1.y, r.e1[2] = e1.z;
+  r.e2[0] = e2.x, r.e2[1] = e2.y, r.e2[2] = e2.z;
+  r.flags = flags;
+  return r;
+}
+
+static void push_pair(Scene &s, const V3 *p, int n) {
+  s.tri_pts.push_back(tri_pts(p[0], p[1], p[2], 0));
+  if (n == 4) {
+    s.tri_pts.push_back(tri_pts(p[1], p[2], p[3], 0));
+  } else {
+    TriPts none{};
+    none.flags = TRIPTS_ABSENT;
+    s.tri_pts.push_back(none);
+  }
   PairPts pp{};
   const V3 q[4] = {p[0], p[1], p[2], n == 4 ? p[3] : p[2]};
   for (int c = 0; c < 3; c++) {
@@ -37,7 +55,6 @@
                         c == 0 ? q[2].x : c == 1 ? q[2].y : q[2].z, c == 0 ? q[3].x : c == 1 ? q[3].y : q[3].z};
     pp.p0[c] = x[0], pp.p1[c] = x[1], pp.p2[c] = x[2], pp.p3[c] = x[3];
   }
-  pp.flags = flags;
   PairBox bx{};
   float diag = 0.f, mag = 0.f;
   for (int c = 0; c < 3; c++) {
@@ -66,7 +83,7 @@
   out.push_back(first);
   out.push_back(second);
   const V3 q[4] = {p0, p1, p2, p3};
-  push_pair(s, q, 4, PAIR_SECOND | ((second.flags & TRI_SAME_E2) ? PAIR_SAME_E2 : 0));
+  push_pair(s, q, 4);
 }
 
 void box_from_points(const V3 p[4], V3 out[8]) {
@@ -494,7 +511,7 @@
 }
 
 std::string Scene::flatten() {
-  pair_boxes.clear(), pair_pts.clear(), tri_nrm.clear(), list_mag = 0.f;
+  pair_boxes.clear(), pair_pts.clear(), tri_pts.clear(), tri_nrm.clear(), list_mag = 0.f;
   sph_groups.clear(), sph_members.clear(), sph_mag = 0.f;
   sliver_faces = 0;
   runs.clear(), spheres.clear(), tris.clear(), bvh_recs.clear(), face_of_orig.clear(), nodes.clear(), qnodes.clear(), faces.clear(), leaf_paths.clear(), tops.clear(),
@@ -572,7 +589,7 @@
         if (!check_mat(ob.mat)) return "triangle without a valid material";
         tris.push_back(hot_tri(ob.p[0], ob.p[1], ob.p[2], ob.mat, 0));
         tris.push_back(HotTri{});
-        push_pair(*this, ob.p, 3, 0);
+        push_pair(*this, ob.p, 3);
         push_run(RUN_TRIS, (int)tris.size() - 2);
         name_pairs(QHIT_TRIANGLE);
         features |= F_TRIS;
@@ -814,6 +831,13 @@
     }
     if (!(mag <= list_mag)) return "margin budget: list_mag is below a pair's coordinates";
   }
+  if (tri_pts.size() != 2 * pair_pts.size() || tris.size() < tri_pts.size()) return "world list: triangle records out of step";
+  for (size_t t = 0; t < tri_pts.size(); t++) {
+    const bool absent = (t & 1) && !(tris[t].flags & TRI_SECOND);
+    if (absent != ((tri_pts[t].flags & TRIPTS_ABSENT) != 0)) return "world list: a triangle record's absent flag is wrong";
+    if (!absent && memcmp(tri_pts[t].p0, tris[t].p0, 9 * sizeof(float)) != 0)
+      return "world list: a triangle record's base point or edges differ from its HotTri's";
+  }
   for (size_t g = 0; g + 1 < sph_groups.size(); g++) {
     const SphGroup &gr = sph_groups[g];
     float mn[3] = {INFINITY, INFINITY, INFINITY}, mx[3] = {-INFINITY, -INFINITY, -INFINITY};
diff --git a/ray-tracing-cuda_amd/csrc/scene_dev.h b/ray-tracing-cuda_amd/csrc/scene_dev.h
--- a/ray-tracing-cuda_amd/csrc/scene_dev.h
+++ b/ray-tracing-cuda_amd/csrc/scene_dev.h
@@ -52,16 +52,17 @@
   int32_t pad[2];
 };
 
-enum : int32_t { PAIR_SECOND = 1, PAIR_SAME_E2 = 2 };
+enum : int32_t { TRIPTS_ABSENT = 1 };
 struct PairBox {
   float mn[3], mx[3];
   int32_t pad[2];
 };
-struct alignas(16) PairPts {
-  float p0[3], p1[3], p2[3], p3[3];
+struct alignas(16) TriPts {
+  float p0[3], e1[3], e2[3];
   int32_t flags;
-  int32_t pad[3];
-};
+  int32_t pad[2];
+};
+static_assert(sizeof(TriPts) == 48, "TriPts is read with three ds_read_b128");
 struct alignas(16) TriNrm {
   float n[3];
   int32_t mat_flags;
@@ -171,7 +172,7 @@
   const SphMember *sph_members;
   float sph_mag;
   int32_t n_sph_groups;
-  const PairPts *pair_pts;
+  const TriPts *tri_pts;
   const TriNrm *tri_nrm;
   const BvhRec *bvhs;
   const BvhNode *nodes;
diff --git a/ray-tracing-cuda_amd/rtmi/__init__.py b/ray-tracing-cuda_amd/rtmi/__init__.py
--- a/ray-tracing-cuda_amd/rtmi/__init__.py
+++ b/ray-tracing-cuda_amd/rtmi/__init__.py
@@ -559,6 +559,19 @@
         keys = ["world", "spheres", "parallelograms", "triangles", "bvh_faces", "bvh_nodes", "materials", "textures"]
         return dict(zip(keys, list(out)))
 
+    def list_records(self):
+        fn = self.L.rtmi_debug_list_records
+        fn.restype, fn.argtypes = C.c_int64, [C.c_void_p, C.c_int64, _u32p, _u32p, _fp]
+        n = _check(fn(self.h, 0, None, None, None), "rtmi_debug_list_records")
+        tp, ht, co = np.zeros((n, 2, 12), np.uint32), np.zeros((n, 2, 16), np.uint32), np.zeros((n, 4, 3), np.float32)
+        _check(fn(self.h, n, tp.ctypes.data_as(_u32p), ht.ctypes.data_as(_u32p), co.ctypes.data_as(_fp)), "rtmi_debug_list_records")
+        return tp, ht, co
+
+    def render_lds_bytes(self, max_depth, threads=256):
+        fn = self.L.rtmi_debug_render_lds_bytes
+        fn.restype, fn.argtypes = C.c_int64, [C.c_void_p, C.c_int, C.c_int]
+        return _check(fn(self.h, max_depth, threads), "rtmi_debug_render_lds_bytes")
+
     def sliver_faces(self):
         return _check(self.L.rtmi_scene_sliver_faces(self.h), "rtmi_scene_sliver_faces")
 
```

Result: faster. 33160 (median of 6 runs) (+1.5%).
